# YangXiaocui1215/MGNNS

Measured on AMD Instinct MI355X. Metric: forward samples/sec at batch 256 (3-channel GCN + fusion), higher is better.
Workload: dtype bf16; 1 GPU; mvsa_multiple_b256: B=256/GPU, T=100, V=20154, 8 heads x 2 layers, C=(80,365), fp32 feature maps [B,2048,14,14] resident in HBM; global_batch=256, parallelism=batch-shard x1, launch=hipGraph replay [segments] x 2 in flight (own buffers, round robin, no join), attention=faithful, forwards_in_flight=2, schedule=place_bank_first

## Files before the change

include/mgnns_hip.h:

```cpp
#ifndef MGNNS_HIP_H
#define MGNNS_HIP_H

#include <stddef.h>
#include <stdint.h>

#ifdef __cplusplus
extern "C" {
#endif

typedef void* mgnns_stream_t;
typedef struct mgnns_comm_s* mgnns_comm_t;

#define MGNNS_ACT_NONE   0
#define MGNNS_ACT_RELU   1
#define MGNNS_ACT_LRELU2 2

#define MGNNS_ERR_ARG     (-1)
#define MGNNS_ERR_LAUNCH  (-2)
#define MGNNS_ERR_UNSUPP  (-3)

#define MGNNS_STATUS_LABEL_GCN_TIMEOUT 1
#define MGNNS_STATUS_CLUSTER_TIMEOUT   2
#define MGNNS_STATUS_BAD_PLAN          3
int mgnns_set_status_word(int32_t* host_pinned);
int mgnns_take_status(void);

const char* mgnns_last_error(void);
#define MGNNS_ABI_VERSION 26
int mgnns_abi_version(void);
const char* mgnns_source_fingerprint(void);
int mgnns_xcd_probe(int32_t* out9);

int mgnns_textgcn_fwd(const int64_t* tok, int B, int T,
                      const float* node_hidden, int V, int D,
                      const float* edge_w, int n_edge_w,
                      const int32_t* pmi_row_ptr, const int32_t* pmi_col, const int32_t* pmi_eid,
                      int ngram, int max_length, float* out, mgnns_stream_t stream);
int mgnns_textgcn_set_form(int form);

int mgnns_embedding_fwd(const int64_t* idx, int64_t n, const float* table, int V, int D,
                        float* out, mgnns_stream_t stream);

size_t mgnns_bilstm_workspace_bytes(int B, int T, int hidden, int num_layers);
int mgnns_bilstm_fwd(const int64_t* tok, const int64_t* lens, int B, int T,
                     const float* emb_table, int V, int emb_dim, int hidden, int num_layers,
                     const float* const* w_ih_cat, const float* const* b_ih_cat,
                     const float* const* w_hh, const float* const* b_hh,
                     void* workspace, size_t workspace_bytes, float* out, void* out_bf16, int ld_bf16,
                     mgnns_stream_t stream);
int mgnns_bilstm_bf16_fwd(const int64_t* tok, const int64_t* lens, int B, int T,
                     const float* emb_table, int V, int emb_dim, int hidden, int num_layers,
                     const float* const* w_ih_cat, const float* const* b_ih_cat,
                     const float* const* w_hh, const float* const* b_hh,
                     void* workspace, size_t workspace_bytes, float* out, void* out_bf16, int ld_bf16, const void* prepacked,
                     mgnns_stream_t stream);
size_t mgnns_bilstm_bf16_prepack_bytes(int hidden, int num_layers);
int mgnns_bilstm_bf16_prepack(const float* const* w_ih_cat, const float* const* w_hh, int emb_dim, int hidden, int num_layers,
                              void* packed, mgnns_stream_t stream);
size_t mgnns_bilstm_bf16_table_bytes(int V, int hidden);
size_t mgnns_bilstm_bf16_fold_workspace_bytes(int V);
int mgnns_bilstm_bf16_fold_embedding(const float* emb_table, int V, int emb_dim, int hidden, const float* w_ih_cat0,
                                     const float* b_ih_cat0, void* workspace, size_t workspace_bytes, float* table,
                                     mgnns_stream_t stream);
int mgnns_bilstm_bf16_table_fwd(const int64_t* tok, const int64_t* lens, int B, int T,
                     const float* emb_table, int V, int emb_dim, int hidden, int num_layers,
                     const float* const* w_ih_cat, const float* const* b_ih_cat,
                     const float* const* w_hh, const float* const* b_hh,
                     void* workspace, size_t workspace_bytes, float* out, void* out_bf16, int ld_bf16, const void* prepacked,
                     const float* gx_table, mgnns_stream_t stream);

int mgnns_gen_adj(const float* A, int C, float* adj, float* work ,
                  int32_t* csr_row_ptr, int32_t* csr_col, float* csr_val, mgnns_stream_t stream);

int mgnns_dense_to_csr(const float* M, int C, int32_t* csr_row_ptr, int32_t* csr_col, float* csr_val,
                       mgnns_stream_t stream);

int mgnns_matmul_fwd(const float* X, int M, int K, const float* W, int N, float* Y, int act,
                     void* workspace, size_t workspace_bytes, mgnns_stream_t stream);
int mgnns_spmm_csr_fwd(const int32_t* row_ptr, const int32_t* col, const float* val, int n_rows,
                       const float* X, int F, float* Y, int act, mgnns_stream_t stream);
int mgnns_spmm_csr_bias_fwd(const int32_t* row_ptr, const int32_t* col, const float* val, int n_rows,
                            const float* X, int F, const float* bias, float* Y, int act, mgnns_stream_t stream);

int mgnns_cast_bf16(const float* src, long long n, void* dst_bf16, mgnns_stream_t stream);
int mgnns_spmm_csr_bf16_fwd(const int32_t* row_ptr, const int32_t* col, const void* val_bf16, int n_rows, int nnz,
                            const void* X_bf16, int F, void* Y, int y_bf16, int act, int variant,
                            const int32_t* row_map, mgnns_stream_t stream);
int mgnns_spmm_tiled_bf16_fwd(const uint32_t* wave_off, const uint32_t* ent, int lane_bytes, int rows_per_wave,
                              int tile_cols, int n_rows, int n_cols, const void* X_bf16, int F, void* Y, int y_bf16,
                              int act, mgnns_stream_t stream);

int mgnns_linear_fwd(const float* X, int M, int K, const float* W, const float* bias, int N,
                     const float* residual, float* Y, int act,
                     void* workspace, size_t workspace_bytes, mgnns_stream_t stream);
size_t mgnns_gemm_workspace_bytes(void);

int mgnns_imgbank_pool_fwd(const float* feat, int B, int K, int P,
                           const float* Wt, int ldw, const float* bias, int N,
                           float* bank, float* pooled, mgnns_stream_t stream);
int mgnns_imgbank_set_form(int form);
size_t mgnns_imgbank_packed_weight_bytes(int K);
int mgnns_imgbank_pack_weights_bf16(const float* W, int N, int K, void* Wp, mgnns_stream_t stream);
int mgnns_imgbank_pool_bf16_fwd(const float* feat, int B, int K, int P, const void* Wp, const float* bias, int N,
                                void* bank_bf16, int ld, float* pooled, float* pooled_work, mgnns_stream_t stream);

int mgnns_imgbank_pool_split_fwd(const float* feat, int B, int K, int P, const void* Wp_hi, const void* Wp_lo,
                                 const float* bias, int N, float* bank, float* pooled_halves, void* bank_hi, void* bank_lo,
                                 mgnns_stream_t stream);

int mgnns_transpose_pad(const float* in, int rows, int cols, float* out, int ld, mgnns_stream_t stream);

int mgnns_label_attn_core_fwd(const float* Q, const float* K, const float* V, int B, int NLQ,
                              int n_heads, int dh, float* x, mgnns_stream_t stream);
int mgnns_label_attn_core_masked_fwd(const float* Q, const float* K, const float* V, const unsigned char* mask,
                                     int B, int NLQ, int n_heads, int dh, float* x, mgnns_stream_t stream);

int mgnns_label_tail_fwd(const float* x, int B, int C, const float* pooled, int n_parts, int K_pool,
                         const float* g_wp, const float* Q, int NLQ, int n_heads, int dh,
                         const float* wk_wp, const float* bk, const float* wv_wp, const float* bv,
                         const float* wc_wp, const float* bc, int N5, const float* xl_wp, const float* bxl,
                         int n_out, float* out, const float* wq_next_wp, const float* bq_next, int HK_next,
                         float* qh_next, mgnns_stream_t stream);

int mgnns_label_tail_bf16_fwd(const float* pooled, int B, int n_parts, int K_pool, int C, int terms,
                              const void* const* packed, const float* Q, int NLQ, int n_heads, int dh, const float* bk,
                              const float* bv, const float* bc, int N5, const float* bxl, int n_out, float* out,
                              const float* bq_next, int HK_next, float* qh_next, float* cluster_scratch,
                              int* cluster_counters, mgnns_stream_t stream);

int mgnns_sq_mha_core_fwd(const float* qh, const float* bank, const float* mask,
                          int B, int L, int D, int H, int dk,
                          const float* Wk, const float* bk, const float* Wv, const float* bv,
                          float* o, float* attn, mgnns_stream_t stream);

int mgnns_head_diff_fwd(const float* o, int B, int H, int dv, float* out, mgnns_stream_t stream);

size_t mgnns_sq_mha_packed_weight_bytes(int H);
int mgnns_sq_mha_pack_weights_bf16(const float* Wk, const float* Wv, int H, int dk, int D, void* Wp,
                                   mgnns_stream_t stream);
int mgnns_cast_pad_bf16(const float* x, int64_t rows, int D, int ld, void* y, mgnns_stream_t stream);
int mgnns_sq_mha_core_bf16_fwd(const float* qh, const void* bank_bf16, const float* mask,
                               int B, int L, int ld, int H, int dk,
                               const void* Wp, const float* bk, const float* bv,
                               float* o, float* attn, mgnns_stream_t stream);

size_t mgnns_sq_mha32_packed_weight_bytes(int H);
int mgnns_sq_mha32_pack_weights_bf16(const float* Wk, const float* Wv, int H, int dk, int D, void* Wp,
                                     mgnns_stream_t stream);
size_t mgnns_sq_mha32_plan_ints(int B);
int mgnns_sq_mha32_plan(const float* mask, int B, int L, int32_t* plan, mgnns_stream_t stream);
int mgnns_sq_mha32_core_bf16_fwd(const float* qh, const void* bank_bf16, const float* mask,
                                 int B, int L, int ld, int H, int dk,
                                 const void* Wp, const float* bk, const float* bv,
                                 float* o, float* attn, const int32_t* plan, mgnns_stream_t stream);

size_t mgnns_sq_mha_split_packed_weight_bytes(int H);
int mgnns_sq_mha_pack_weights_split(const float* Wk, const float* Wv, int H, int dk, int D, void* Wp,
                                    mgnns_stream_t stream);
int mgnns_split_pad_bf16(const float* x, int64_t rows, int D, int ld, void* hi, void* lo, mgnns_stream_t stream);
int mgnns_sq_mha_core_split_fwd(const float* qh, const void* bank_hi, const void* bank_lo, const float* mask,
                                int B, int L, int ld, int H, int dk,
                                const void* Wp, const float* bk, const float* bv,
                                float* o, float* attn, const int32_t* plan, mgnns_stream_t stream);
int mgnns_sq_mha_split_plan(const float* mask, int B, int L, int32_t* plan, mgnns_stream_t stream);

size_t mgnns_sq_mha_folded_workspace_bytes(int B, int D, int H);
int mgnns_sq_mha_folded_fwd(const float* qh, const void* bank, int bank_is_bf16, int ld_bank, const float* mask,
                            int B, int L, int D, int H, int dk, const float* Wk, const float* Wv, const float* bv,
                            void* workspace, size_t workspace_bytes, float* o, float* attn, mgnns_stream_t stream);

int mgnns_sq_mha_folded_bf16_fwd(const float* U, const void* bank_bf16, const float* mask, int B, int L, int D, int H,
                                 float inv_temp, void* C_bf16, int ldc, float* attn, mgnns_stream_t stream);

size_t mgnns_packed_f32_weight_bytes(int N, int K);
int mgnns_pack_weight_f32(const float* W, int N, int K, float* Wp, mgnns_stream_t stream);
int mgnns_mha_tail_fwd(const float* o, int HK, const float* q, int B, int d_model,
                       const float* fc_wp, const float* fc_b, const float* ln1_gamma, const float* ln1_beta,
                       const float* w1_wp, const float* b1, const float* w2_wp, const float* b2,
                       const float* ln2_gamma, const float* ln2_beta, float eps, float* out,
                       const float* wq_next_wp, const float* bq_next, int HK_next, float* qh_next,
                       mgnns_stream_t stream);

size_t mgnns_packed_bf16_weight_bytes(int N, int K);
int mgnns_pack_weight_bf16_split(const float* W, int N, int K, void* Whi, void* Wlo, mgnns_stream_t stream);
int mgnns_mha_tail_bf16_fwd(const float* o, int HK, const float* q, int B, int d_model, int terms,
                            const void* const* packed,
                            const float* fc_b, const float* ln1_gamma, const float* ln1_beta, const float* b1,
                            const float* b2, const float* ln2_gamma, const float* ln2_beta, float eps, float* out,
                            const float* bq_next, int HK_next, float* qh_next, int cluster, float* cluster_scratch,
                            int* cluster_counters, mgnns_stream_t stream);

size_t mgnns_mha_tail_c16_scratch_floats(int B, int cluster);
int mgnns_mha_tail_c16_fwd(const void* c_bf16, int HC, const float* q, int B, int d_model, const void* const* packed,
                           const float* fc_b, const float* ln1_gamma, const float* ln1_beta, const float* b1,
                           const float* b2, const float* ln2_gamma, const float* ln2_beta, float eps, float* out,
                           const float* bq_next, int HC_next, float* u_next, int cluster, float* cluster_scratch,
                           int* cluster_counters, mgnns_stream_t stream);

int mgnns_label_gcn_supported(int C, int K0, int N1, int N2, int split);
int mgnns_label_tail_supported(int C, int NLQ, int n_heads, int dh, int N5, int n_out, int K_pool, int with_next_q);
int mgnns_label_tail_bf16_supported(int C, int NLQ, int n_heads, int dh, int N5, int n_out, int K_pool, int terms, int with_next_q);
size_t mgnns_label_gcn_scratch_bytes(int C, int N1, int N2);
int mgnns_label_gcn_fwd(const float* A, int C, const float* inp, int K0, int split, const void* w1a, const void* w1b, int N1,
                        const void* w2a, const void* w2b, int N2, float* G, void* Gp_hi, void* Gp_lo,
                        const float* label_query, int NLQ, const float* wq, const float* bq, int HQ, float* Q,
                        void* scratch, size_t scratch_bytes, int grid, mgnns_stream_t stream);
size_t mgnns_label_gcn_memo_bytes(int C, int K0);
int mgnns_label_gcn_memo_fwd(const float* A, int C, const float* inp, int K0, int split, const void* w1a, const void* w1b, int N1,
                             const void* w2a, const void* w2b, int N2, float* G, void* Gp_hi, void* Gp_lo,
                             const float* label_query, int NLQ, const float* wq, const float* bq, int HQ, float* Q,
                             void* scratch, size_t scratch_bytes, void* memo, size_t memo_bytes, int grid, mgnns_stream_t stream);

int mgnns_classifier_head_fwd(const float* f0, const float* f1, const float* f2, const float* f3, int B, int D,
                              const float* W, const float* bias, int NL, float* logits, mgnns_stream_t stream);
int mgnns_classifier_part_fwd(const float* f, int part, int nparts, int B, int D, const float* W, const float* bias,
                              int NL, float* parts, int* counter, float* logits, mgnns_stream_t stream);

int mgnns_layernorm_fwd(const float* x, int rows, int D, const float* gamma, const float* beta,
                        float eps, float* y, mgnns_stream_t stream);

int mgnns_mha_train_fwd(const float* qh, const float* bank, const float* mask, int B, int L, int D, int H, int dk,
                        const float* Wk, const float* Wv, const float* bv, uint64_t seed, float rate, float* U, float* P,
                        float* attn, uint8_t* keep, float* Z, float* SP, float* o, mgnns_stream_t stream);
size_t mgnns_mha_train_bwd_workspace_bytes(int B, int D, int H, int dk);
int mgnns_mha_train_bwd(const float* dO, const float* qh, const float* bank, const float* mask, int B, int L, int D, int H,
                        int dk, const float* Wk, const float* Wv, const float* bv, float rate, const float* U, const float* P,
                        const float* attn, const uint8_t* keep, const float* Z, const float* SP, float* dqh, float* dWk,
                        float* dWv, float* dbv, float* dbank, void* workspace, size_t workspace_bytes, mgnns_stream_t stream);
size_t mgnns_wgrad_workspace_bytes(int M, int N, int K);
int mgnns_wgrad_fwd(const float* dY, int M, int N, const float* X, int K, float* dW, float* db, void* workspace,
                    size_t workspace_bytes, mgnns_stream_t stream);
int mgnns_drop_res_ln_fwd(const float* x, const float* res, int rows, int D, const float* gamma, const float* beta, float eps,
                          uint64_t seed, int site, float rate, float* y, float* xhat, float* sig, uint8_t* keep,
                          mgnns_stream_t stream);
int mgnns_drop_res_ln_bwd(const float* dy, const float* dy2, const float* xhat, const float* sig, const uint8_t* keep, int rows,
                          int D, const float* gamma, float eps, float rate, float* dres, float* dx, float* dgamma, float* dbeta,
                          mgnns_stream_t stream);
#define MGNNS_ELT_ADD        0
#define MGNNS_ELT_RELU_BWD   1
#define MGNNS_ELT_LRELU2_BWD 2
int mgnns_train_eltwise(int op, const float* a, const float* b, int64_t n, float* y, mgnns_stream_t stream);

#define MGNNS_DROP_LABEL_ATTN 3
#define MGNNS_DROP_HEAD       4
size_t mgnns_imgbank_wgrad_workspace_bytes(int B, int K, int P, int N);
int mgnns_imgbank_wgrad(const float* X, const float* dbank, int B, int K, int P, int N, float* dW, float* db, void* workspace,
                        size_t workspace_bytes, mgnns_stream_t stream);
int mgnns_map_argmax(const float* X, int B, int K, int P, int32_t* arg, mgnns_stream_t stream);
int mgnns_imgbank_dgrad(const float* dbank, const float* W, const float* dpooled, const int32_t* arg, int B, int K, int P, int N,
                        float* dX, mgnns_stream_t stream);
size_t mgnns_imgbank_wgrad_split_workspace_bytes(int B, int K, int P, int N);
int mgnns_imgbank_wgrad_split(const float* X, const float* dbank, int B, int K, int P, int N, float* dW, float* db,
                              void* workspace, size_t workspace_bytes, mgnns_stream_t stream);
size_t mgnns_imgbank_dgrad_split_workspace_bytes(int B, int K, int P, int N);
int mgnns_imgbank_dgrad_split(const float* dbank, const float* W, const float* dpooled, const int32_t* arg, int B, int K, int P,
                              int N, float* dX, void* workspace, size_t workspace_bytes, mgnns_stream_t stream);
int mgnns_label_attn_train_fwd(const float* Q, const float* K, const float* V, int B, int NLQ, int H, int dh, uint64_t seed,
                               float rate, float* x, float* P, uint8_t* keep, mgnns_stream_t stream);
size_t mgnns_label_attn_train_bwd_workspace_bytes(int B, int NLQ, int H, int dh);
int mgnns_label_attn_train_bwd(const float* dx, const float* Q, const float* K, const float* V, const float* P,
                               const uint8_t* keep, int B, int NLQ, int H, int dh, float rate, float* dQ, float* dK, float* dV,
                               void* workspace, size_t workspace_bytes, mgnns_stream_t stream);

#define MGNNS_DROP_LSTM       5
#define MGNNS_DROP_TEXT_GCN   6
size_t mgnns_bilstm_train_workspace_bytes(int B, int T, int hidden);
int mgnns_bilstm_train_fwd(const int64_t* tok, const int64_t* lens, int B, int T, const float* emb_table, int V, int emb_dim,
                           int hidden, int num_layers, const float* const* w_ih_cat, const float* const* b_ih_cat,
                           const float* const* w_hh, const float* const* b_hh, uint64_t seed, float rate, int32_t* meta,
                           int rows_cap, float* gates, float* cells, float* mid, float* mid_drop, float* out, void* workspace,
                           size_t workspace_bytes, mgnns_stream_t stream);
int mgnns_bilstm_train_bwd_rec(const float* dout, const int64_t* lens, int B, int T, const int32_t* meta, int rows_cap,
                               const float* gates, const float* cells, const float* w_hh_f, const float* w_hh_r, float* dz,
                               mgnns_stream_t stream);
int mgnns_bilstm_train_hprev(const float* hout, const int64_t* lens, int B, int T, const int32_t* meta, int rows_cap, float* hprev,
                             mgnns_stream_t stream);
int mgnns_bilstm_train_unpack_drop(const float* dx, const int32_t* pack_pos, int64_t M, int B, int T, uint64_t seed, float rate,
                                   float* dout, mgnns_stream_t stream);
int mgnns_gather_rows(const float* src, int n_src, int K, const int32_t* idx, int64_t M, float* dst, mgnns_stream_t stream);
int mgnns_keyed_row_sum(const int64_t* sorted_keys, const int64_t* perm, int64_t M, const float* values, int D, int64_t n_values,
                        int64_t skip_below, float* out, int64_t K, mgnns_stream_t stream);
int mgnns_textgcn_train_fwd(const int64_t* tok, int B, int T, const float* node_hidden, int V, int D, const float* edge_w,
                            int n_edge_w, const int32_t* pmi_row_ptr, const int32_t* pmi_col, const int32_t* pmi_eid, int ngram,
                            int max_length, uint64_t seed, float rate, float* out, float* presum, int16_t* win,
                            mgnns_stream_t stream);
int mgnns_textgcn_train_bwd(const int64_t* tok, int B, int T, const float* node_hidden, int V, int D, const float* edge_w,
                            int n_edge_w, const int32_t* pmi_row_ptr, const int32_t* pmi_col, const int32_t* pmi_eid, int ngram,
                            int max_length, uint64_t seed, float rate, const float* dy, const float* presum, const int16_t* win,
                            float* R, int32_t* keyR, float* Eg, int32_t* keyE, mgnns_stream_t stream);
int mgnns_dropout_fwd(const float* x, int64_t n, uint64_t seed, int site, float rate, float* y, uint8_t* keep,
                      mgnns_stream_t stream);
int mgnns_dropout_bwd(const float* dy, const uint8_t* keep, int64_t n, float rate, float* dx, mgnns_stream_t stream);
int mgnns_dropout_mask(uint64_t seed, int site, float rate, int64_t n, uint8_t* keep, mgnns_stream_t stream);

int mgnns_transpose_cast_bf16(const float* x, int rows, int cols, int ld, void* y, mgnns_stream_t stream);
size_t mgnns_gemm_bf16_workspace_bytes(void);
int mgnns_gemm_bf16_nt_fwd(const void* A, const void* Bt, int M, int N, int Kp, const float* bias, void* C, int ldc,
                           int c_bf16, int act, void* workspace, size_t workspace_bytes, mgnns_stream_t stream);
int mgnns_gemm_bf16_set_form(int form);
int mgnns_gemm_bf16_pick_form(int M, int N, int Kp, int with_workspace, int n_cu);

int mgnns_softmax_argmax_fwd(const float* logits, int B, int NL, float* probs, int32_t* pred, const int64_t* target,
                             int32_t* confusion, mgnns_stream_t stream);

int mgnns_conv_fold_bn_bf16(const float* w, const float* conv_bias, int Cout, int Cin, int KH, int KW,
                            const float* gamma, const float* beta, const float* mean, const float* var, float eps,
                            int k_order, int ld, void* wt, float* bias, mgnns_stream_t stream);
int mgnns_stem_conv7_fwd(const float* img, int B, int H, int W, const void* wt, const float* bias, void* y,
                         mgnns_stream_t stream);
int mgnns_maxpool3x3s2_nhwc_fwd(const void* x, int B, int H, int W, int C, void* y, mgnns_stream_t stream);
int mgnns_conv_bf16_nhwc_fwd(const void* x, int B, int H, int W, int Cin, const void* wt, const float* bias, int Cout,
                             int KH, int KW, int stride, int pad, const void* residual, int relu, int out_nchw_f32,
                             void* y, mgnns_stream_t stream);

int mgnns_conv_transpose_pack_bf16(const void* wt, int Cout, int Cin, int KH, int KW, void* wT, mgnns_stream_t stream);
int mgnns_conv_dgrad_bf16_nhwc(const void* dy, int B, int H, int W, int Cin, const void* wT, int Cout, int KH, int KW,
                               int stride, int pad, const void* mask, const void* add, void* dx, mgnns_stream_t stream);
size_t mgnns_conv_wgrad_workspace_bytes(int B, int H, int W, int Cin, int Cout, int KH, int KW, int stride, int pad);
int mgnns_conv_wgrad_bf16_nhwc(const void* x, const void* dy, int B, int H, int W, int Cin, int Cout, int KH, int KW,
                               int stride, int pad, float* dW, float* db, void* workspace, size_t workspace_bytes,
                               mgnns_stream_t stream);
int mgnns_conv_bn_unfold(const float* dWp, const float* dbp, const float* w, const float* gamma, const float* mean,
                         const float* var, float eps, int Cout, int Cin, int KH, int KW, float* dW, float* dgamma,
                         float* dbeta, mgnns_stream_t stream);
int mgnns_map_grad_relu_nhwc_bf16(const float* map, const float* dmap, int B, int C, int P, void* g, mgnns_stream_t stream);

size_t mgnns_bn_stats_workspace_bytes(int M, int C);
int mgnns_bn_stats_bf16(const void* z, int M, int C, float eps, double momentum, float* mean, float* rstd, float* var,
                        float* running_mean, float* running_var, void* workspace, size_t workspace_bytes,
                        mgnns_stream_t stream);
int mgnns_bn_apply_bf16(const void* z, int M, int C, const float* mean, const float* rstd, const float* gamma,
                        const float* beta, const void* residual, int relu, int out_nchw_f32, int P, void* y,
                        mgnns_stream_t stream);
size_t mgnns_bn_backward_workspace_bytes(int M, int C);
int mgnns_bn_backward_bf16(const void* g, const void* z, int M, int C, const float* mean, const float* rstd,
                           const float* gamma, void* gz, float* dgamma, float* dbeta, void* workspace,
                           size_t workspace_bytes, mgnns_stream_t stream);

int mgnns_debug_stamp(uint64_t* slots, int idx, mgnns_stream_t stream);

int mgnns_debug_slabcopy(const void* src, void* dst, int n_rows, int pitch, int piece, int mode, int wgx,
                         mgnns_stream_t stream);

int mgnns_debug_spin(int microseconds, uint64_t* slots, int idx, mgnns_stream_t stream);

int mgnns_comm_unique_id(void* id, size_t bytes );
int mgnns_comm_init_rank(int world, int rank, const void* id, size_t bytes, mgnns_comm_t* comm);
int mgnns_comm_init_all(int ndev, const int* devices, mgnns_comm_t* comms);
int mgnns_comm_info(mgnns_comm_t comm, int* world, int* rank);
int mgnns_allgather_logits(mgnns_comm_t comm, const float* local, int rows_local, int num_labels, float* all,
                           mgnns_stream_t stream);
int mgnns_comm_group_start(void);
int mgnns_comm_group_end(void);
int mgnns_comm_destroy(mgnns_comm_t comm);

#ifdef __cplusplus
}
#endif
#endif
```

mgnns_amd/_lib.py:

```python
import ctypes
import os

_HERE = os.path.dirname(os.path.abspath(__file__))
LIB_PATH = os.environ.get("MGNNS_LIB") or os.path.join(_HERE, "libmgnns_hip.so")
ABI_VERSION = 26

_c = ctypes
_P = _c.c_void_p
_I = _c.c_int
_L = _c.c_int64
_F = _c.c_float
_SZ = _c.c_size_t
_U64 = _c.c_uint64
_PP = _c.POINTER(_c.c_void_p)

SIGNATURES = {
    "mgnns_textgcn_fwd": [_P, _I, _I, _P, _I, _I, _P, _I, _P, _P, _P, _I, _I, _P, _P],
    "mgnns_bilstm_fwd": [_P, _P, _I, _I, _P, _I, _I, _I, _I, _PP, _PP, _PP, _PP, _P, _SZ, _P, _P, _I, _P],
    "mgnns_bilstm_bf16_fwd": [_P, _P, _I, _I, _P, _I, _I, _I, _I, _PP, _PP, _PP, _PP, _P, _SZ, _P, _P, _I, _P, _P],
    "mgnns_bilstm_bf16_prepack": [_PP, _PP, _I, _I, _I, _P, _P],
    "mgnns_bilstm_bf16_fold_embedding": [_P, _I, _I, _I, _P, _P, _P, _SZ, _P, _P],
    "mgnns_bilstm_bf16_table_fwd": [_P, _P, _I, _I, _P, _I, _I, _I, _I, _PP, _PP, _PP, _PP, _P, _SZ, _P, _P, _I, _P, _P, _P],
    "mgnns_embedding_fwd": [_P, _L, _P, _I, _I, _P, _P],
    "mgnns_gen_adj": [_P, _I, _P, _P, _P, _P, _P, _P],
    "mgnns_dense_to_csr": [_P, _I, _P, _P, _P, _P],
    "mgnns_matmul_fwd": [_P, _I, _I, _P, _I, _P, _I, _P, _SZ, _P],
    "mgnns_spmm_csr_fwd": [_P, _P, _P, _I, _P, _I, _P, _I, _P],
    "mgnns_spmm_csr_bias_fwd": [_P, _P, _P, _I, _P, _I, _P, _P, _I, _P],
    "mgnns_cast_bf16": [_P, _c.c_longlong, _P, _P],
    "mgnns_spmm_csr_bf16_fwd": [_P, _P, _P, _I, _I, _P, _I, _P, _I, _I, _I, _P, _P],
    "mgnns_spmm_tiled_bf16_fwd": [_P, _P, _I, _I, _I, _I, _I, _P, _I, _P, _I, _I, _P],
    "mgnns_linear_fwd": [_P, _I, _I, _P, _P, _I, _P, _P, _I, _P, _SZ, _P],
    "mgnns_imgbank_pool_fwd": [_P, _I, _I, _I, _P, _I, _P, _I, _P, _P, _P],
    "mgnns_imgbank_pack_weights_bf16": [_P, _I, _I, _P, _P],
    "mgnns_imgbank_pool_bf16_fwd": [_P, _I, _I, _I, _P, _P, _I, _P, _I, _P, _P, _P],
    "mgnns_imgbank_set_form": [_I],
    "mgnns_textgcn_set_form": [_I],
    "mgnns_head_diff_fwd": [_P, _I, _I, _I, _P, _P],
    "mgnns_classifier_part_fwd": [_P, _I, _I, _I, _I, _P, _P, _I, _P, _P, _P, _P],
    "mgnns_imgbank_pool_split_fwd": [_P, _I, _I, _I, _P, _P, _P, _I, _P, _P, _P, _P, _P],
    "mgnns_transpose_pad": [_P, _I, _I, _P, _I, _P],
    "mgnns_label_attn_core_fwd": [_P, _P, _P, _I, _I, _I, _I, _P, _P],
    "mgnns_label_attn_core_masked_fwd": [_P, _P, _P, _P, _I, _I, _I, _I, _P, _P],
    "mgnns_label_gcn_fwd": [_P, _I, _P, _I, _I, _P, _P, _I, _P, _P, _I, _P, _P, _P, _P, _I, _P, _P, _I, _P, _P, _SZ, _I, _P],
    "mgnns_label_gcn_memo_fwd": [_P, _I, _P, _I, _I, _P, _P, _I, _P, _P, _I, _P, _P, _P, _P, _I, _P, _P, _I, _P, _P, _SZ, _P, _SZ, _I, _P],
    "mgnns_classifier_head_fwd": [_P, _P, _P, _P, _I, _I, _P, _P, _I, _P, _P],
    "mgnns_label_tail_bf16_fwd": [_P, _I, _I, _I, _I, _I, _PP, _P, _I, _I, _I, _P, _P, _P, _I, _P, _I, _P, _P, _I, _P, _P, _P, _P],
    "mgnns_label_tail_fwd": [_P, _I, _I, _P, _I, _I, _P, _P, _I, _I, _I, _P, _P, _P, _P, _P, _P, _I, _P, _P, _I, _P, _P, _P,
                             _I, _P, _P],
    "mgnns_sq_mha_core_fwd": [_P, _P, _P, _I, _I, _I, _I, _I, _P, _P, _P, _P, _P, _P, _P],
    "mgnns_sq_mha_pack_weights_bf16": [_P, _P, _I, _I, _I, _P, _P],
    "mgnns_cast_pad_bf16": [_P, _L, _I, _I, _P, _P],
    "mgnns_sq_mha_core_bf16_fwd": [_P, _P, _P, _I, _I, _I, _I, _I, _P, _P, _P, _P, _P, _P],
    "mgnns_sq_mha32_pack_weights_bf16": [_P, _P, _I, _I, _I, _P, _P],
    "mgnns_sq_mha32_plan": [_P, _I, _I, _P, _P],
    "mgnns_sq_mha32_core_bf16_fwd": [_P, _P, _P, _I, _I, _I, _I, _I, _P, _P, _P, _P, _P, _P, _P],
    "mgnns_sq_mha_pack_weights_split": [_P, _P, _I, _I, _I, _P, _P],
    "mgnns_split_pad_bf16": [_P, _L, _I, _I, _P, _P, _P],
    "mgnns_sq_mha_core_split_fwd": [_P, _P, _P, _P, _I, _I, _I, _I, _I, _P, _P, _P, _P, _P, _P, _P],
    "mgnns_sq_mha_split_plan": [_P, _I, _I, _P, _P],
    "mgnns_sq_mha_folded_fwd": [_P, _P, _I, _I, _P, _I, _I, _I, _I, _I, _P, _P, _P, _P, _SZ, _P, _P, _P],
    "mgnns_pack_weight_f32": [_P, _I, _I, _P, _P],
    "mgnns_mha_tail_fwd": [_P, _I, _P, _I, _I, _P, _P, _P, _P, _P, _P, _P, _P, _P, _P, _F, _P, _P, _P, _I, _P, _P],
    "mgnns_pack_weight_bf16_split": [_P, _I, _I, _P, _P, _P],
    "mgnns_mha_tail_bf16_fwd": [_P, _I, _P, _I, _I, _I, _PP, _P, _P, _P, _P, _P, _P, _P, _F, _P, _P, _I, _P, _I, _P, _P, _P],
    "mgnns_mha_tail_c16_fwd": [_P, _I, _P, _I, _I, _PP, _P, _P, _P, _P, _P, _P, _P, _F, _P, _P, _I, _P, _I, _P, _P, _P],
    "mgnns_sq_mha_folded_bf16_fwd": [_P, _P, _P, _I, _I, _I, _I, _F, _P, _I, _P, _P],
    "mgnns_transpose_cast_bf16": [_P, _I, _I, _I, _P, _P],
    "mgnns_gemm_bf16_nt_fwd": [_P, _P, _I, _I, _I, _P, _P, _I, _I, _I, _P, _SZ, _P],
    "mgnns_gemm_bf16_set_form": [_I],
    "mgnns_gemm_bf16_pick_form": [_I, _I, _I, _I, _I],
    "mgnns_softmax_argmax_fwd": [_P, _I, _I, _P, _P, _P, _P, _P],
    "mgnns_conv_fold_bn_bf16": [_P, _P, _I, _I, _I, _I, _P, _P, _P, _P, _F, _I, _I, _P, _P, _P],
    "mgnns_stem_conv7_fwd": [_P, _I, _I, _I, _P, _P, _P, _P],
    "mgnns_maxpool3x3s2_nhwc_fwd": [_P, _I, _I, _I, _I, _P, _P],
    "mgnns_conv_bf16_nhwc_fwd": [_P, _I, _I, _I, _I, _P, _P, _I, _I, _I, _I, _I, _P, _I, _I, _P, _P],
    "mgnns_conv_transpose_pack_bf16": [_P, _I, _I, _I, _I, _P, _P],
    "mgnns_conv_dgrad_bf16_nhwc": [_P, _I, _I, _I, _I, _P, _I, _I, _I, _I, _I, _P, _P, _P, _P],
    "mgnns_conv_wgrad_bf16_nhwc": [_P, _P, _I, _I, _I, _I, _I, _I, _I, _I, _I, _P, _P, _P, _SZ, _P],
    "mgnns_conv_bn_unfold": [_P, _P, _P, _P, _P, _P, _F, _I, _I, _I, _I, _P, _P, _P, _P],
    "mgnns_map_grad_relu_nhwc_bf16": [_P, _P, _I, _I, _I, _P, _P],
    "mgnns_bn_stats_bf16": [_P, _I, _I, _F, _c.c_double, _P, _P, _P, _P, _P, _P, _SZ, _P],
    "mgnns_bn_apply_bf16": [_P, _I, _I, _P, _P, _P, _P, _P, _I, _I, _I, _P, _P],
    "mgnns_bn_backward_bf16": [_P, _P, _I, _I, _P, _P, _P, _P, _P, _P, _P, _SZ, _P],
    "mgnns_label_gcn_supported": [_I, _I, _I, _I, _I],
    "mgnns_label_tail_supported": [_I, _I, _I, _I, _I, _I, _I, _I],
    "mgnns_label_tail_bf16_supported": [_I, _I, _I, _I, _I, _I, _I, _I, _I],
    "mgnns_xcd_probe": [_P],
    "mgnns_set_status_word": [_P],
    "mgnns_take_status": [],
    "mgnns_debug_slabcopy": [_P, _P, _I, _I, _I, _I, _I, _P],
    "mgnns_debug_stamp": [_P, _I, _P],
    "mgnns_debug_spin": [_I, _P, _I, _P],
    "mgnns_layernorm_fwd": [_P, _I, _I, _P, _P, _F, _P, _P],
    "mgnns_mha_train_fwd": [_P, _P, _P, _I, _I, _I, _I, _I, _P, _P, _P, _U64, _F, _P, _P, _P, _P, _P, _P, _P, _P],
    "mgnns_mha_train_bwd": [_P, _P, _P, _P, _I, _I, _I, _I, _I, _P, _P, _P, _F, _P, _P, _P, _P, _P, _P, _P, _P, _P, _P, _P,
                            _P, _SZ, _P],
    "mgnns_wgrad_fwd": [_P, _I, _I, _P, _I, _P, _P, _P, _SZ, _P],
    "mgnns_drop_res_ln_fwd": [_P, _P, _I, _I, _P, _P, _F, _U64, _I, _F, _P, _P, _P, _P, _P],
    "mgnns_drop_res_ln_bwd": [_P, _P, _P, _P, _P, _I, _I, _P, _F, _F, _P, _P, _P, _P, _P],
    "mgnns_train_eltwise": [_I, _P, _P, _L, _P, _P],
    "mgnns_imgbank_wgrad": [_P, _P, _I, _I, _I, _I, _P, _P, _P, _SZ, _P],
    "mgnns_map_argmax": [_P, _I, _I, _I, _P, _P],
    "mgnns_imgbank_dgrad": [_P, _P, _P, _P, _I, _I, _I, _I, _P, _P],
    "mgnns_imgbank_wgrad_split": [_P, _P, _I, _I, _I, _I, _P, _P, _P, _SZ, _P],
    "mgnns_imgbank_dgrad_split": [_P, _P, _P, _P, _I, _I, _I, _I, _P, _P, _SZ, _P],
    "mgnns_label_attn_train_fwd": [_P, _P, _P, _I, _I, _I, _I, _U64, _F, _P, _P, _P, _P],
    "mgnns_label_attn_train_bwd": [_P, _P, _P, _P, _P, _P, _I, _I, _I, _I, _F, _P, _P, _P, _P, _SZ, _P],
    "mgnns_dropout_fwd": [_P, _L, _U64, _I, _F, _P, _P, _P],
    "mgnns_dropout_bwd": [_P, _P, _L, _F, _P, _P],
    "mgnns_dropout_mask": [_U64, _I, _F, _L, _P, _P],
    "mgnns_bilstm_train_fwd": [_P, _P, _I, _I, _P, _I, _I, _I, _I, _PP, _PP, _PP, _PP, _U64, _F, _P, _I, _P, _P, _P, _P, _P, _P,
                               _SZ, _P],
    "mgnns_bilstm_train_bwd_rec": [_P, _P, _I, _I, _P, _I, _P, _P, _P, _P, _P, _P],
    "mgnns_bilstm_train_hprev": [_P, _P, _I, _I, _P, _I, _P, _P],
    "mgnns_bilstm_train_unpack_drop": [_P, _P, _L, _I, _I, _U64, _F, _P, _P],
    "mgnns_gather_rows": [_P, _I, _I, _P, _L, _P, _P],
    "mgnns_keyed_row_sum": [_P, _P, _L, _P, _I, _L, _L, _P, _L, _P],
    "mgnns_textgcn_train_fwd": [_P, _I, _I, _P, _I, _I, _P, _I, _P, _P, _P, _I, _I, _U64, _F, _P, _P, _P, _P],
    "mgnns_textgcn_train_bwd": [_P, _I, _I, _P, _I, _I, _P, _I, _P, _P, _P, _I, _I, _U64, _F, _P, _P, _P, _P, _P, _P, _P, _P],
    "mgnns_comm_unique_id": [_P, _SZ],
    "mgnns_comm_init_rank": [_I, _I, _P, _SZ, _PP],
    "mgnns_comm_init_all": [_I, _P, _PP],
    "mgnns_comm_info": [_P, _c.POINTER(_I), _c.POINTER(_I)],
    "mgnns_allgather_logits": [_P, _P, _I, _I, _P, _P],
    "mgnns_comm_group_start": [],
    "mgnns_comm_group_end": [],
    "mgnns_comm_destroy": [_P],
}

SIZE_GETTERS = {
    "mgnns_packed_bf16_weight_bytes": [_I, _I],
    "mgnns_packed_f32_weight_bytes": [_I, _I],
    "mgnns_gemm_workspace_bytes": [],
    "mgnns_gemm_bf16_workspace_bytes": [],
    "mgnns_imgbank_packed_weight_bytes": [_I],
    "mgnns_sq_mha_packed_weight_bytes": [_I],
    "mgnns_sq_mha32_packed_weight_bytes": [_I],
    "mgnns_sq_mha32_plan_ints": [_I],
    "mgnns_sq_mha_split_packed_weight_bytes": [_I],
    "mgnns_sq_mha_folded_workspace_bytes": [_I, _I, _I],
    "mgnns_bilstm_workspace_bytes": [_I, _I, _I, _I],
    "mgnns_bilstm_bf16_prepack_bytes": [_I, _I],
    "mgnns_bilstm_bf16_table_bytes": [_I, _I],
    "mgnns_bilstm_bf16_fold_workspace_bytes": [_I],
    "mgnns_label_gcn_scratch_bytes": [_I, _I, _I],
    "mgnns_label_gcn_memo_bytes": [_I, _I],
    "mgnns_mha_tail_c16_scratch_floats": [_I, _I],
    "mgnns_mha_train_bwd_workspace_bytes": [_I, _I, _I, _I],
    "mgnns_wgrad_workspace_bytes": [_I, _I, _I],
    "mgnns_imgbank_wgrad_workspace_bytes": [_I, _I, _I, _I],
    "mgnns_imgbank_wgrad_split_workspace_bytes": [_I, _I, _I, _I],
    "mgnns_imgbank_dgrad_split_workspace_bytes": [_I, _I, _I, _I],
    "mgnns_label_attn_train_bwd_workspace_bytes": [_I, _I, _I, _I],
    "mgnns_bilstm_train_workspace_bytes": [_I, _I, _I],
    "mgnns_conv_wgrad_workspace_bytes": [_I, _I, _I, _I, _I, _I, _I, _I, _I],
    "mgnns_bn_stats_workspace_bytes": [_I, _I],
    "mgnns_bn_backward_workspace_bytes": [_I, _I],
}

_lib = None


class MgnnsLibraryError(RuntimeError):
    pass


def lib():
    global _lib
    if _lib is not None:
        return _lib
    if not os.path.exists(LIB_PATH):
        raise MgnnsLibraryError(
            "%s is missing: the HIP extension is mandatory (no CPU/PyTorch fallback exists). "
            "Build it with `python -m mgnns_amd.build`." % LIB_PATH)
    import torch
    L = ctypes.CDLL(LIB_PATH)
    L.mgnns_last_error.restype = ctypes.c_char_p
    L.mgnns_last_error.argtypes = []
    L.mgnns_abi_version.restype = _I
    L.mgnns_abi_version.argtypes = []
    L.mgnns_source_fingerprint.restype = ctypes.c_char_p
    L.mgnns_source_fingerprint.argtypes = []
    if L.mgnns_abi_version() != ABI_VERSION:
        raise MgnnsLibraryError("libmgnns_hip.so ABI %d != binding ABI %d; rebuild" % (L.mgnns_abi_version(), ABI_VERSION))
    for name, args in SIZE_GETTERS.items():
        fn = getattr(L, name)
        fn.restype = _SZ
        fn.argtypes = args
    for name, args in SIGNATURES.items():
        fn = getattr(L, name)
        fn.restype = _I
        fn.argtypes = args
    _lib = L
    _register_status_word(L)
    return L


def source_state():
    from . import build
    built, tree = lib().mgnns_source_fingerprint().decode(), build.source_fingerprint()
    return built, tree, built == tree


def check_sources(who="this measurement"):
    built, tree, same = source_state()
    if not same:
        raise MgnnsLibraryError("%s: %s was built from sources %s, the tree holds %s -- rebuild (python -m mgnns_amd.build) first"
                                % (who, LIB_PATH, built, tree))
    return built


_status_word = None


def _register_status_word(L):
    global _status_word
    import torch
    if _status_word is not None or not torch.cuda.is_available():
        return
    try:
        w = torch.zeros(16, dtype=torch.int32).pin_memory()
    except RuntimeError:
        return
    L.mgnns_set_status_word(w.data_ptr())
    _status_word = w


def xcd_probe():
    import ctypes
    out = (ctypes.c_int32 * 9)()
    check(lib().mgnns_xcd_probe(ctypes.addressof(out)), "mgnns_xcd_probe")
    return bool(out[0]), [int(out[1 + k]) for k in range(8)]


def take_status():
    code = lib().mgnns_take_status()
    if code:
        raise RuntimeError("a launch raised the library status word (status %d: 1 / 2 = a persistent launch gave up a bounded wait, "
                           "3 = a masked attention launch refused its plan): results since then are invalid" % code)


def check(rc, name):
    if rc != 0:
        raise RuntimeError("%s failed (%d): %s" % (name, rc, lib().mgnns_last_error().decode()))
```

mgnns_amd/csrc/label_tail.hip:

```cpp
#include "common.hpp"
#include "tile_f32.hpp"

namespace {

constexpr int LT_THR = 512;
constexpr int LT_ROWS = 16;
constexpr int LT_MAXKQ = 20;
constexpr int LT_MAXH = 8;

__host__ __device__ inline int lt_stride(int k) {
    const int kp = (k + 15) / 16 * 16;
    return kp + ((34 - (kp % 32)) % 32);
}

constexpr int LT_KCH = 512;

__global__ __launch_bounds__(LT_THR) void label_tail_kernel(const float* __restrict__ x, int B, int C,
                                                            const float* __restrict__ pooled, int n_parts, int KP,
                                                            const float* __restrict__ g_wp,
                                                            const float* __restrict__ Q, int NLQ, int n_heads, int dh,
                                                            const float* __restrict__ wk_wp, const float* __restrict__ bk,
                                                            const float* __restrict__ wv_wp, const float* __restrict__ bv,
                                                            const float* __restrict__ wc_wp, const float* __restrict__ bc, int N5,
                                                            const float* __restrict__ xl_wp, const float* __restrict__ bxl, int NO,
                                                            float* __restrict__ out, const float* __restrict__ wq_wp,
                                                            const float* __restrict__ bq, int HKn, float* __restrict__ qh_next) {
    extern __shared__ __attribute__((aligned(16))) float smem[];
    const int hid = n_heads * dh;
    const int sx = lt_stride(C), sh = lt_stride(hid), sf = lt_stride(NLQ * N5);
    float* s_x = smem;
    float* s_k = s_x + LT_ROWS * sx;
    float* s_v = s_k + LT_ROWS * sh;
    float* s_o = s_v + LT_ROWS * sh;
    float* s_f = s_o + LT_ROWS * sh;
    float* s_q = s_f + LT_ROWS * sf;
    const int tid = threadIdx.x, lane = tid & 63, wave = tid >> 6;
    const int r0 = blockIdx.x * LT_ROWS;
    const int crow = (lane >> 4) * 4, ccol = lane & 15;
    const int NTh = (hid + 15) / 16, NT5 = (N5 + 15) / 16, NTo = (NO + 15) / 16;
    const int KQh = (hid + 15) / 16;

    f32x4 wc[LT_MAXKQ];
    if (wave < NT5) {
#pragma unroll
        for (int kq = 0; kq < LT_MAXKQ; ++kq)
            wc[kq] = kq < KQh ? reinterpret_cast<const f32x4*>(wc_wp)[((size_t)wave * KQh + kq) * 64 + lane] : f32x4{0.f, 0.f, 0.f, 0.f};
    }
    for (int i = tid; i < LT_ROWS * sx + 3 * LT_ROWS * sh + LT_ROWS * sf; i += LT_THR) s_x[i] = 0.f;
    for (int i = tid; i < NLQ * hid; i += LT_THR) s_q[i] = Q[i];
    __syncthreads();
    if (g_wp) {
        const int NTc = (C + 15) / 16, KQ = (KP + 15) / 16;
        const int sp = lt_stride(LT_KCH);
        float* s_p = s_f;
        for (int t0 = 0; t0 * 8 < NTc; t0 += 3) {
            f32x4 acc[3] = {f32x4{0.f, 0.f, 0.f, 0.f}, f32x4{0.f, 0.f, 0.f, 0.f}, f32x4{0.f, 0.f, 0.f, 0.f}};
            for (int k0 = 0; k0 < KP; k0 += LT_KCH) {
                const int kn = min(LT_KCH, KP - k0);
                for (int i = tid; i < LT_ROWS * (LT_KCH / 4); i += LT_THR) {
                    const int r = i / (LT_KCH / 4), c4 = (i - r * (LT_KCH / 4)) * 4;
                    f32x4 v = {0.f, 0.f, 0.f, 0.f};
                    if (r0 + r < B && c4 < kn) {
                        const float* src = pooled + ((size_t)(r0 + r) * n_parts) * KP + k0 + c4;
                        v = *reinterpret_cast<const f32x4*>(src);
                        for (int pt = 1; pt < n_parts; ++pt) {
                            const f32x4 u = *reinterpret_cast<const f32x4*>(src + (size_t)pt * KP);
                            v = f32x4{fmaxf(v.x, u.x), fmaxf(v.y, u.y), fmaxf(v.z, u.z), fmaxf(v.w, u.w)};
                        }
                    }
                    float* d = s_p + r * sp + c4;
                    *reinterpret_cast<float2*>(d) = float2{v.x, v.y};
                    *reinterpret_cast<float2*>(d + 2) = float2{v.z, v.w};
                }
                __syncthreads();
                mg_tile_gemm_f32_chunk<3>(acc, s_p, sp, k0 / 16, (k0 + kn + 15) / 16, KQ, g_wp, NTc, wave, lane, t0);
                __syncthreads();
            }
#pragma unroll
            for (int t = 0; t < 3; ++t) {
                const int nt = wave + 8 * (t0 + t), n = nt * 16 + ccol;
                if (nt < NTc && n < C) {
#pragma unroll
                    for (int r = 0; r < 4; ++r) s_x[(crow + r) * sx + n] = acc[t][r];
                }
            }
        }
        for (int i = tid; i < LT_ROWS * sf; i += LT_THR) s_f[i] = 0.f;
    } else {
        for (int i = tid; i < LT_ROWS * C; i += LT_THR) {
            const int r = i / C, c = i - r * C;
            if (r0 + r < B) s_x[r * sx + c] = x[(size_t)(r0 + r) * C + c];
        }
    }
    __syncthreads();

    for (int t0 = 0; t0 * 8 < NTh; t0 += 3) {
        f32x4 ak[3], av[3];
        mg_tile_gemm_f32<3>(ak, s_x, sx, C, wk_wp, NTh, wave, lane, t0);
        mg_tile_gemm_f32<3>(av, s_x, sx, C, wv_wp, NTh, wave, lane, t0);
#pragma unroll
        for (int t = 0; t < 3; ++t) {
            const int nt = wave + 8 * (t0 + t), n = nt * 16 + ccol;
            if (nt < NTh && n < hid) {
                const float b0 = bk[n], b1 = bv[n];
#pragma unroll
                for (int r = 0; r < 4; ++r) {
                    s_k[(crow + r) * sh + n] = ak[t][r] + b0;
                    s_v[(crow + r) * sh + n] = av[t][r] + b1;
                }
            }
        }
    }
    __syncthreads();

    const float inv_scale = 1.0f / sqrtf((float)dh);
    for (int l = 0; l < NLQ; ++l) {
#pragma unroll 1
        for (int rr = 0; rr < 2; ++rr) {
            const int r = 2 * wave + rr;
            const bool on = lane < dh;
            float e[LT_MAXH], vv[LT_MAXH];
#pragma unroll
            for (int h = 0; h < LT_MAXH; ++h) {
                const int c = (h < n_heads ? h : 0) * dh + (on ? lane : 0);
                e[h] = (on && h < n_heads) ? s_q[l * hid + c] * s_k[r * sh + c] * inv_scale : -INFINITY;
                vv[h] = s_v[r * sh + c];
            }
#pragma unroll
            for (int h = 0; h < LT_MAXH; ++h) {
                if (h < n_heads) {
                    const float m = wave_max_dpp(e[h]);
                    const float p = on ? expf(e[h] - m) : 0.f;
                    const float z = wave_sum_dpp(p);
                    if (on) s_o[r * sh + h * dh + lane] = (p / z) * vv[h];
                }
            }
        }
        __syncthreads();
        if (wave < NT5) {
            f32x4 acc = {0.f, 0.f, 0.f, 0.f};
            const float* ap = s_o + (lane & 15) * sh + (lane >> 4);
#pragma unroll
            for (int kq = 0; kq < LT_MAXKQ; ++kq) {
                if (kq < KQh) {
#pragma unroll
                    for (int j = 0; j < 4; ++j) acc = __builtin_amdgcn_mfma_f32_16x16x4f32(ap[(4 * kq + j) * 4], wc[kq][j], acc, 0, 0, 0);
                }
            }
            const int n = wave * 16 + ccol;
            if (n < N5) {
                const float b0 = bc[n];
#pragma unroll
                for (int r = 0; r < 4; ++r) s_f[(crow + r) * sf + l * N5 + n] = acc[r] + b0;
            }
        }
        __syncthreads();
    }

    for (int t0 = 0; t0 * 8 < NTo; t0 += 3) {
        f32x4 acc[3];
        mg_tile_gemm_f32<3>(acc, s_f, sf, NLQ * N5, xl_wp, NTo, wave, lane, t0);
#pragma unroll
        for (int t = 0; t < 3; ++t) {
            const int nt = wave + 8 * (t0 + t), n = nt * 16 + ccol;
            if (nt < NTo && n < NO) {
                const float b0 = bxl[n];
#pragma unroll
                for (int r = 0; r < 4; ++r) {
                    const int gr = r0 + crow + r;
                    const float v = acc[t][r] + b0;
                    if (gr < B) out[(size_t)gr * NO + n] = v;
                    if (wq_wp) s_o[(crow + r) * sh + n] = v;
                }
            }
        }
    }
    if (wq_wp) {
        __syncthreads();
        const int NTq = (HKn + 15) / 16;
        for (int t0 = 0; t0 * 8 < NTq; t0 += 3) {
            f32x4 acc[3];
            mg_tile_gemm_f32<3>(acc, s_o, sh, NO, wq_wp, NTq, wave, lane, t0);
#pragma unroll
            for (int t = 0; t < 3; ++t) {
                const int nt = wave + 8 * (t0 + t), n = nt * 16 + ccol;
                if (nt < NTq && n < HKn) {
                    const float b0 = bq ? bq[n] : 0.f;
#pragma unroll
                    for (int r = 0; r < 4; ++r) {
                        const int gr = r0 + crow + r;
                        if (gr < B) qh_next[(size_t)gr * HKn + n] = acc[t][r] + b0;
                    }
                }
            }
        }
    }
}

}

extern "C" int mgnns_label_tail_supported(int C, int NLQ, int n_heads, int dh, int N5, int n_out, int K_pool, int with_next_q) {
    if (!(C > 0 && NLQ > 0 && n_heads > 0 && dh > 0 && dh <= 64 && N5 > 0 && n_out > 0)) return 0;
    if (K_pool && K_pool % 4) return 0;
    const int hid = n_heads * dh;
    if (!(hid <= 16 * LT_MAXKQ && n_heads <= LT_MAXH && N5 <= 128)) return 0;
    if (with_next_q && n_out != hid) return 0;
    if (K_pool && lt_stride(NLQ * N5) < lt_stride(LT_KCH)) return 0;
    const size_t lds = ((size_t)LT_ROWS * (lt_stride(C) + 3 * lt_stride(hid) + lt_stride(NLQ * N5)) + (size_t)NLQ * hid) * sizeof(float);
    return lds <= 160 * 1024 ? 1 : 0;
}

extern "C" int mgnns_label_tail_fwd(const float* x, int B, int C, const float* pooled, int n_parts, int K_pool,
                                    const float* g_wp, const float* Q, int NLQ, int n_heads, int dh,
                                    const float* wk_wp, const float* bk, const float* wv_wp, const float* bv,
                                    const float* wc_wp, const float* bc, int N5, const float* xl_wp, const float* bxl,
                                    int n_out, float* out, const float* wq_next_wp, const float* bq_next, int HK_next,
                                    float* qh_next, mgnns_stream_t stream) {
    MG_REQUIRE(B >= 0 && C > 0 && NLQ > 0 && n_heads > 0 && dh > 0 && dh <= 64 && N5 > 0 && n_out > 0,
               "mgnns_label_tail_fwd: bad dims B=%d C=%d NLQ=%d heads=%d dh=%d N5=%d out=%d", B, C, NLQ, n_heads, dh, N5, n_out);
    if (B == 0) return 0;
    MG_REQUIRE(Q && wk_wp && bk && wv_wp && bv && wc_wp && bc && xl_wp && bxl && out, "mgnns_label_tail_fwd: null pointer");
    MG_REQUIRE((x != nullptr) != (g_wp != nullptr), "mgnns_label_tail_fwd: pass EITHER the read-out x OR pooled + packed G");
    if (g_wp) {
        MG_REQUIRE(pooled && n_parts >= 1 && K_pool > 0 && K_pool % 4 == 0 && mg_aligned16(pooled),
                   "mgnns_label_tail_fwd: pooled [B,%d,%d] must be 16-byte aligned with K %% 4 == 0", n_parts, K_pool);
    }
    const int hid = n_heads * dh;
    MG_REQUIRE(hid <= 16 * LT_MAXKQ && n_heads <= LT_MAXH, "mgnns_label_tail_fwd: hidden width %d / %d heads unsupported (<= %d, <= %d)",
               hid, n_heads, 16 * LT_MAXKQ, LT_MAXH);
    MG_REQUIRE(N5 <= 128, "mgnns_label_tail_fwd: linear_5 width %d unsupported (<= 128)", N5);
    MG_REQUIRE(!wq_next_wp || (qh_next && HK_next > 0 && n_out == hid),
               "mgnns_label_tail_fwd: the query projection needs qh_next, HK_next and n_out == hidden width");
    const int sfl = lt_stride(NLQ * N5) > lt_stride(LT_KCH) || !g_wp ? lt_stride(NLQ * N5) : lt_stride(LT_KCH);
    MG_REQUIRE(!g_wp || lt_stride(NLQ * N5) >= lt_stride(LT_KCH), "mgnns_label_tail_fwd: NLQ*N5=%d too small to stage the read-out (>= %d)",
               NLQ * N5, LT_KCH);
    (void)sfl;
    const size_t lds = ((size_t)LT_ROWS * (lt_stride(C) + 3 * lt_stride(hid) + lt_stride(NLQ * N5)) + (size_t)NLQ * hid) * sizeof(float);
    MG_REQUIRE(lds <= 160 * 1024, "mgnns_label_tail_fwd: C=%d, NLQ*N5=%d need %zu B of LDS (> 160 KiB)", C, NLQ * N5, lds);
    MG_DYN_LDS(label_tail_kernel, 160 * 1024);
    hipLaunchKernelGGL(label_tail_kernel, dim3((B + LT_ROWS - 1) / LT_ROWS), dim3(LT_THR), lds, (hipStream_t)stream, x, B, C,
                       pooled, n_parts, K_pool, g_wp, Q, NLQ, n_heads, dh, wk_wp, bk, wv_wp, bv, wc_wp, bc, N5, xl_wp, bxl, n_out,
                       out, wq_next_wp, bq_next, HK_next, qh_next);
    MG_CHECK_LAUNCH("mgnns_label_tail_fwd");
    return 0;
}

#include "tile_bf16.hpp"

#ifdef MG_LT_TRACE
__device__ unsigned long long g_lt_trace[16];
#define LT_STAMP(i) do { if (threadIdx.x == 0 && blockIdx.x == 0) g_lt_trace[i] = __builtin_amdgcn_s_memtime(); } while (0)
extern "C" int mgnns_debug_lt_trace(unsigned long long* out) {
    return hipMemcpyFromSymbol(out, HIP_SYMBOL(g_lt_trace), sizeof(unsigned long long) * 16) == hipSuccess ? 0 : 1;
}
#else
#define LT_STAMP(i) do { } while (0)
#endif

namespace {

constexpr int LB_MAXKS = 10;

struct LabelW {
    const unsigned short *g_h, *g_l, *wk_h, *wk_l, *wv_h, *wv_l, *wc_h, *wc_l, *xl_h, *xl_l, *wq_h, *wq_l;
    const float *bk, *bv, *bc, *bxl, *bq;
};

__device__ __forceinline__ unsigned pk2(float a, float b) { return mg_bf16(a) | (unsigned)mg_bf16(b) << 16; }

template <int TERMS, int CL>
__global__ __launch_bounds__(LT_THR) void label_tail_bf16_kernel(const float* __restrict__ pooled, int B, int n_parts, int KP, int C,
                                                                 const float* __restrict__ Q, int NLQ, int n_heads, int dh,
                                                                 LabelW w, int N5, int NO, float* __restrict__ out, int HKn,
                                                                 float* __restrict__ qh_next, float* __restrict__ xpart,
                                                                 int* __restrict__ counters, int* __restrict__ status) {
    extern __shared__ __attribute__((aligned(16))) unsigned char smem_b[];
    constexpr int NH = TERMS == 3 ? 4 : 1;
    constexpr int LO = TERMS == 3 ? 1 : 0;
    const int hid = n_heads * dh;
    const int KSp = KP / 32, KSpp = KSp / NH, KSx = (C + 31) / 32, KSh = (hid + 31) / 32, KSf = (NLQ * N5 + 31) / 32;
    const int sp = 4 * KSpp + 2, sxc = 4 * KSx + 2, shc = 4 * KSh + 2, sfc = 4 * KSf + 2;
    const int shf = lt_stride(hid);
    const int spf = sp > sfc ? sp : sfc;
    uint4* s_ph = reinterpret_cast<uint4*>(smem_b);
    uint4* s_pl = s_ph + LT_ROWS * spf;
    uint4* s_xh = s_pl + LO * LT_ROWS * spf;
    uint4* s_xl = s_xh + LT_ROWS * sxc;
    uint4* s_oh = s_xl + LO * LT_ROWS * sxc;
    uint4* s_ol = s_oh + LT_ROWS * shc;
    float* s_k = reinterpret_cast<float*>(s_ol + LO * LT_ROWS * shc);
    float* s_v = s_k + LT_ROWS * shf;
    float* s_q = s_v + LT_ROWS * shf;
    uint4* s_fh = s_ph;
    uint4* s_fl = s_pl;
    if (!LO) { s_pl = s_ph; s_xl = s_xh; s_ol = s_oh; s_fl = s_fh; }
    const int tid = threadIdx.x, lane = tid & 63, wave = tid >> 6;
    const int tile = (int)blockIdx.x / CL, crank = (int)blockIdx.x % CL;
    const int r0 = tile * LT_ROWS;
    const int crow = (lane >> 4) * 4, ccol = lane & 15;
    const int NTc = (C + 15) / 16, NTh = (hid + 15) / 16, NT5 = (N5 + 15) / 16, NTo = (NO + 15) / 16;
    unsigned short* xh16 = reinterpret_cast<unsigned short*>(s_xh);
    unsigned short* xl16 = reinterpret_cast<unsigned short*>(s_xl);
    unsigned short* oh16 = reinterpret_cast<unsigned short*>(s_oh);
    unsigned short* ol16 = reinterpret_cast<unsigned short*>(s_ol);
    unsigned short* fh16 = reinterpret_cast<unsigned short*>(s_fh);
    unsigned short* fl16 = reinterpret_cast<unsigned short*>(s_fl);
    auto put = [&](unsigned short* h, unsigned short* l, int idx, float v) {
        if (LO) mg_split_store(h, l, idx, v); else h[idx] = mg_bf16(v);
    };

    LT_STAMP(0);
#ifndef MG_LT_TOUCH
#define MG_LT_TOUCH 0
#endif
#ifndef MG_LT_PF3
#define MG_LT_PF3 4
#endif
    WRing<3, TERMS, (TERMS == 3 ? MG_LT_PF3 : 10)> ring;
    ring_prime(ring, KSpp, w.g_h, w.g_l, NTc, wave, lane, 0, KSp, CL > 1 ? crank * KSpp : 0);
#if MG_LT_TOUCH
    int touch_sink = 0;
    {
        auto touch = [&](const unsigned short* base, int nt_n, int ks_total, int ks_lo, int ks_n, int nt_lo = 0) {
            if (!base || nt_n <= 0) return;
            base += ((size_t)nt_lo * ks_total) << 9;
            const int lines = nt_n * ks_n * 8;
            for (int i = tid; i < lines; i += LT_THR) {
                const int nt = i / (ks_n * 8), rem = i - nt * (ks_n * 8);
                const char* p = reinterpret_cast<const char*>(base) + ((size_t)(nt * ks_total + ks_lo + (rem >> 3)) << 10) + ((rem & 7) << 7);
                asm volatile("global_load_dword %0, %1, off" : "+v"(touch_sink) : "v"(p) : "memory");
            }
        };
        const int NTq_ = (HKn + 15) / 16;
        touch(w.g_h, NTc, KSp, CL > 1 ? crank * KSpp : 0, CL > 1 ? KSpp : KSp);
        if (LO) touch(w.g_l, NTc, KSp, CL > 1 ? crank * KSpp : 0, CL > 1 ? KSpp : KSp);
        touch(w.wk_h, NTh, KSx, 0, KSx);
        if (LO) touch(w.wk_l, NTh, KSx, 0, KSx);
        touch(w.wv_h, NTh, KSx, 0, KSx);
        if (LO) touch(w.wv_l, NTh, KSx, 0, KSx);
        touch(w.wc_h, NT5, KSh, 0, KSh);
        if (LO) touch(w.wc_l, NT5, KSh, 0, KSh);
        touch(w.xl_h, NTo, KSf, 0, KSf);
        if (LO) touch(w.xl_l, NTo, KSf, 0, KSf);
        const int qs_ = (NTq_ + 7) / 8, qp_ = (qs_ + CL - 1) / CL;
        const int qt_lo = crank * qp_ * 8, qt_hi = (crank * qp_ + qp_) * 8 < NTq_ ? (crank * qp_ + qp_) * 8 : NTq_;
        touch(w.wq_h, qt_hi - qt_lo, KSh, 0, KSh, qt_lo);
        if (LO) touch(w.wq_l, qt_hi - qt_lo, KSh, 0, KSh, qt_lo);
    }
#endif
    for (int i = tid; i < (1 + LO) * LT_ROWS * (sxc + shc); i += LT_THR) s_xh[i] = make_uint4(0u, 0u, 0u, 0u);
    for (int i = tid; i < 2 * LT_ROWS * shf; i += LT_THR) s_k[i] = 0.f;
    for (int i = tid; i < NLQ * hid; i += LT_THR) s_q[i] = Q[i];

    f32x4 acc[3];
    LT_STAMP(1);
    static_assert(CL == 1 || CL == NH, "a cluster rank owns one K part of the read-out");
    for (int hpart = CL > 1 ? crank : 0; hpart < (CL > 1 ? crank + 1 : NH); ++hpart) {
        const int kq8 = KP / NH / 8;
        for (int i = tid; i < LT_ROWS * kq8; i += LT_THR) {
            const int r = i / kq8, c8 = i - r * kq8;
            f32x4 a = {0.f, 0.f, 0.f, 0.f}, b = a;
            if (r0 + r < B) {
                const float* src = pooled + ((size_t)(r0 + r) * n_parts) * KP + hpart * (KP / NH) + 8 * c8;
                a = *reinterpret_cast<const f32x4*>(src);
                b = *reinterpret_cast<const f32x4*>(src + 4);
                for (int pt = 1; pt < n_parts; ++pt) {
                    const f32x4 u = *reinterpret_cast<const f32x4*>(src + (size_t)pt * KP);
                    const f32x4 v = *reinterpret_cast<const f32x4*>(src + (size_t)pt * KP + 4);
                    a = f32x4{fmaxf(a.x, u.x), fmaxf(a.y, u.y), fmaxf(a.z, u.z), fmaxf(a.w, u.w)};
                    b = f32x4{fmaxf(b.x, v.x), fmaxf(b.y, v.y), fmaxf(b.z, v.z), fmaxf(b.w, v.w)};
                }
            }
            s_ph[r * sp + c8] = make_uint4(pk2(a.x, a.y), pk2(a.z, a.w), pk2(b.x, b.y), pk2(b.z, b.w));
            if (LO) {
                auto lo = [](float x) { return x - mg_bf16_f32(mg_bf16(x)); };
                s_pl[r * sp + c8] = make_uint4(pk2(lo(a.x), lo(a.y)), pk2(lo(a.z), lo(a.w)), pk2(lo(b.x), lo(b.y)), pk2(lo(b.z), lo(b.w)));
            }
        }
        __syncthreads();
        if (CL == 1 && hpart) ring_prime(ring, KSpp, w.g_h, w.g_l, NTc, wave, lane, 0, KSp, hpart * KSpp);
        ring_gemm(acc, ring, s_ph, s_pl, sp, KSpp, w.g_h, w.g_l, lane, CL == 1 && hpart != 0);
        __syncthreads();
    }
    LT_STAMP(2);
    ring_prime(ring, KSx, w.wk_h, w.wk_l, NTh, wave, lane, 0);
    if (CL > 1) {
        const __amdgpu_buffer_rsrc_t xp = mg_buffer(xpart + (size_t)tile * CL * (8 * 3 * 64 * 4), CL * 8 * 3 * 64 * 16);
        const int slot = (wave * 3 * 64 + lane) * 16;
#pragma unroll
        for (int t = 0; t < 3; ++t)
            if (wave + 8 * t < NTc)
                __builtin_amdgcn_raw_buffer_store_b128(__builtin_bit_cast(i32x4, acc[t]), xp, slot + t * 64 * 16, crank * (8 * 3 * 64 * 16), 17);
        asm volatile("s_waitcnt vmcnt(0)" ::: "memory");
        __syncthreads();
        if (tid == 0) {
            __hip_atomic_fetch_add(&counters[2 * tile], 1, __ATOMIC_RELAXED, __HIP_MEMORY_SCOPE_AGENT);
            int spins = 0;
            while (__hip_atomic_load(&counters[2 * tile], __ATOMIC_RELAXED, __HIP_MEMORY_SCOPE_AGENT) < CL) {
                if (++spins > (1 << 24)) {
                    if (status) __hip_atomic_store(status, MGNNS_STATUS_CLUSTER_TIMEOUT, __ATOMIC_RELAXED, __HIP_MEMORY_SCOPE_SYSTEM);
                    break;
                }
                __builtin_amdgcn_s_sleep(4);
            }
        }
        __syncthreads();
#pragma unroll
        for (int t = 0; t < 3; ++t) {
            f32x4 pr[CL];
#pragma unroll
            for (int rk = 0; rk < CL; ++rk)
                pr[rk] = wave + 8 * t < NTc ? __builtin_bit_cast(f32x4, __builtin_amdgcn_raw_buffer_load_b128(xp, slot + t * 64 * 16, rk * (8 * 3 * 64 * 16), 17))
                                            : f32x4{0.f, 0.f, 0.f, 0.f};
            acc[t] = pr[0];
#pragma unroll
            for (int rk = 1; rk < CL; ++rk) acc[t] += pr[rk];
        }
    }
#pragma unroll
    for (int t = 0; t < 3; ++t) {
        const int nt = wave + 8 * t, n = nt * 16 + ccol;
        if (nt < NTc && n < C) {
#pragma unroll
            for (int r = 0; r < 4; ++r) put(xh16, xl16, (crow + r) * sxc * 8 + n, acc[t][r]);
        }
    }
    for (int i = tid; i < (1 + LO) * LT_ROWS * spf; i += LT_THR) s_ph[i] = make_uint4(0u, 0u, 0u, 0u);
    __syncthreads();
    if (CL > 1 && tid == 0) {
        const int old = __hip_atomic_fetch_add(&counters[2 * tile + 1], 1, __ATOMIC_RELAXED, __HIP_MEMORY_SCOPE_AGENT);
        if (old == CL - 1) {
            __hip_atomic_store(&counters[2 * tile], 0, __ATOMIC_RELAXED, __HIP_MEMORY_SCOPE_AGENT);
            __hip_atomic_store(&counters[2 * tile + 1], 0, __ATOMIC_RELAXED, __HIP_MEMORY_SCOPE_AGENT);
        }
    }
    LT_STAMP(3);
    ring_gemm(acc, ring, s_xh, s_xl, sxc, KSx, w.wk_h, w.wk_l, lane);
    ring_prime(ring, KSx, w.wv_h, w.wv_l, NTh, wave, lane, 0);
#pragma unroll
    for (int t = 0; t < 3; ++t) {
        const int nt = wave + 8 * t, n = nt * 16 + ccol;
        if (nt < NTh && n < hid) {
            const float b0 = w.bk[n];
#pragma unroll
            for (int r = 0; r < 4; ++r) s_k[(crow + r) * shf + n] = acc[t][r] + b0;
        }
    }
    ring_gemm(acc, ring, s_xh, s_xl, sxc, KSx, w.wv_h, w.wv_l, lane);
    ring_prime(ring, KSf, w.xl_h, w.xl_l, NTo, wave, lane, 0);
#pragma unroll
    for (int t = 0; t < 3; ++t) {
        const int nt = wave + 8 * t, n = nt * 16 + ccol;
        if (nt < NTh && n < hid) {
            const float b0 = w.bv[n];
#pragma unroll
            for (int r = 0; r < 4; ++r) s_v[(crow + r) * shf + n] = acc[t][r] + b0;
        }
    }
    uint4 wch[LB_MAXKS], wcl[LO ? LB_MAXKS : 1];
    if (wave < NT5) {
#pragma unroll
        for (int ks = 0; ks < LB_MAXKS; ++ks) {
            const size_t off = ((size_t)wave * KSh + (ks < KSh ? ks : 0)) * 64 + lane;
            wch[ks] = reinterpret_cast<const uint4*>(w.wc_h)[off];
            if (LO) wcl[ks] = reinterpret_cast<const uint4*>(w.wc_l)[off];
        }
    }
    __syncthreads();

    const float inv_scale = 1.0f / sqrtf((float)dh);
    LT_STAMP(4);
    for (int l = 0; l < NLQ; ++l) {
#pragma unroll 1
        for (int rr = 0; rr < 2; ++rr) {
            const int r = 2 * wave + rr;
            const bool on = lane < dh;
            float e[LT_MAXH], vv[LT_MAXH];
#pragma unroll
            for (int h = 0; h < LT_MAXH; ++h) {
                const int c = (h < n_heads ? h : 0) * dh + (on ? lane : 0);
                e[h] = (on && h < n_heads) ? s_q[l * hid + c] * s_k[r * shf + c] * inv_scale : -INFINITY;
                vv[h] = s_v[r * shf + c];
            }
#pragma unroll
            for (int h = 0; h < LT_MAXH; ++h) {
                if (h < n_heads) {
                    const float m = wave_max_dpp(e[h]);
                    const float p = on ? __expf(e[h] - m) : 0.f;
                    const float z = wave_sum_dpp(p);
                    if (on) put(oh16, ol16, r * shc * 8 + h * dh + lane, (p / z) * vv[h]);
                }
            }
        }
        __syncthreads();
        if (wave < NT5) {
            f32x4 a = {0.f, 0.f, 0.f, 0.f};
            const int aoff = (lane & 15) * shc + (lane >> 4);
#pragma unroll
            for (int ks = 0; ks < LB_MAXKS; ++ks)
                if (ks < KSh) {
                    const bf16x8 ah = __builtin_bit_cast(bf16x8, s_oh[aoff + ks * 4]);
                    a = __builtin_amdgcn_mfma_f32_16x16x32_bf16(ah, __builtin_bit_cast(bf16x8, wch[ks]), a, 0, 0, 0);
                    if (LO) {
                        a = __builtin_amdgcn_mfma_f32_16x16x32_bf16(ah, __builtin_bit_cast(bf16x8, wcl[ks]), a, 0, 0, 0);
                        a = __builtin_amdgcn_mfma_f32_16x16x32_bf16(__builtin_bit_cast(bf16x8, s_ol[aoff + ks * 4]),
                                                                    __builtin_bit_cast(bf16x8, wch[ks]), a, 0, 0, 0);
                    }
                }
            const int n = wave * 16 + ccol;
            if (n < N5) {
                const float b0 = w.bc[n];
#pragma unroll
                for (int r = 0; r < 4; ++r) put(fh16, fl16, (crow + r) * sfc * 8 + l * N5 + n, a[r] + b0);
            }
        }
        __syncthreads();
    }

    LT_STAMP(5);
    ring_gemm(acc, ring, s_fh, s_fl, sfc, KSf, w.xl_h, w.xl_l, lane);
    LT_STAMP(6);
    const int q_slots = ((HKn + 15) / 16 + 7) / 8, q_per = (q_slots + CL - 1) / CL;
    const int q_lo = crank * q_per, q_hi = q_lo + q_per < q_slots ? q_lo + q_per : q_slots;
    if (w.wq_h) ring_prime(ring, KSh, w.wq_h, w.wq_l, (HKn + 15) / 16, wave, lane, q_lo);
#pragma unroll
    for (int t = 0; t < 3; ++t) {
        const int nt = wave + 8 * t, n = nt * 16 + ccol;
        if (nt < NTo && n < NO) {
            const float b0 = w.bxl[n];
#pragma unroll
            for (int r = 0; r < 4; ++r) {
                const int gr = r0 + crow + r;
                const float v = acc[t][r] + b0;
                if (gr < B && crank == 0) out[(size_t)gr * NO + n] = v;
                if (w.wq_h) put(oh16, ol16, (crow + r) * shc * 8 + n, v);
            }
        }
    }
    if (w.wq_h) {
        __syncthreads();
        const int NTq = (HKn + 15) / 16;
        for (int t0 = q_lo; t0 < q_hi; t0 += 3) {
            if (t0 != q_lo) ring_prime(ring, KSh, w.wq_h, w.wq_l, NTq, wave, lane, t0);
            ring_gemm(acc, ring, s_oh, s_ol, shc, KSh, w.wq_h, w.wq_l, lane);
#pragma unroll
            for (int t = 0; t < 3; ++t) {
                const int nt = wave + 8 * (t0 + t), n = nt * 16 + ccol;
                if (t0 + t < q_hi && nt < NTq && n < HKn) {
                    const float b0 = w.bq ? w.bq[n] : 0.f;
#pragma unroll
                    for (int r = 0; r < 4; ++r) {
                        const int gr = r0 + crow + r;
                        if (gr < B) qh_next[(size_t)gr * HKn + n] = acc[t][r] + b0;
                    }
                }
            }
        }
    }
#if MG_LT_TOUCH
    asm volatile("s_waitcnt vmcnt(0)" : "+v"(touch_sink)::"memory");
#endif
    LT_STAMP(7);
}

}

extern "C" int mgnns_label_tail_bf16_supported(int C, int NLQ, int n_heads, int dh, int N5, int n_out, int K_pool, int terms,
                                               int with_next_q) {
    if (!(C > 0 && C <= 384 && NLQ > 0 && n_heads > 0 && dh > 0 && dh <= 64 && N5 > 0 && N5 <= 128 && n_out > 0)) return 0;
    if (terms != 1 && terms != 3) return 0;
    if (!(K_pool > 0 && K_pool % 128 == 0)) return 0;
    const int hid = n_heads * dh;
    if (!(hid <= 32 * LB_MAXKS && n_out <= 384 && n_heads <= LT_MAXH)) return 0;
    if (with_next_q && n_out != hid) return 0;
    const int nh = terms == 3 ? 4 : 1, lo = terms == 3 ? 1 : 0;
    const int sp = 4 * (K_pool / 32 / nh) + 2, sxc = 4 * ((C + 31) / 32) + 2, shc = 4 * ((hid + 31) / 32) + 2, sfc = 4 * ((NLQ * N5 + 31) / 32) + 2;
    const size_t lds = (size_t)(1 + lo) * LT_ROWS * ((sp > sfc ? sp : sfc) + sxc + shc) * 16 +
                       ((size_t)2 * LT_ROWS * lt_stride(hid) + (size_t)NLQ * hid) * sizeof(float);
    return lds <= 160 * 1024 ? 1 : 0;
}

extern "C" int mgnns_label_tail_bf16_fwd(const float* pooled, int B, int n_parts, int K_pool, int C, int terms,
                                         const void* const* packed ,
                                         const float* Q, int NLQ, int n_heads, int dh, const float* bk, const float* bv,
                                         const float* bc, int N5, const float* bxl, int n_out, float* out,
                                         const float* bq_next, int HK_next, float* qh_next, float* cluster_scratch,
                                         int* cluster_counters, mgnns_stream_t stream) {
    MG_REQUIRE(B >= 0 && C > 0 && C <= 384 && NLQ > 0 && n_heads > 0 && dh > 0 && dh <= 64 && N5 > 0 && N5 <= 128 && n_out > 0,
               "mgnns_label_tail_bf16_fwd: bad dims B=%d C=%d (<= 384) NLQ=%d heads=%d dh=%d N5=%d out=%d", B, C, NLQ, n_heads, dh, N5, n_out);
    MG_REQUIRE(terms == 1 || terms == 3, "mgnns_label_tail_bf16_fwd: terms must be 1 (bf16) or 3 (split-bf16)");
    if (B == 0) return 0;
    MG_REQUIRE(pooled && packed && Q && bk && bv && bc && bxl && out, "mgnns_label_tail_bf16_fwd: null pointer");
    for (int i = 0; i < 10; ++i) MG_REQUIRE(packed[i], "mgnns_label_tail_bf16_fwd: packed weight %d missing", i);
    MG_REQUIRE(n_parts >= 1 && K_pool > 0 && K_pool % 128 == 0 && mg_aligned16(pooled),
               "mgnns_label_tail_bf16_fwd: pooled [B,%d,%d] must be 16-byte aligned with K %% 128 == 0", n_parts, K_pool);
    const int hid = n_heads * dh;
    MG_REQUIRE(hid <= 32 * LB_MAXKS && n_out <= 384 && n_heads <= LT_MAXH,
               "mgnns_label_tail_bf16_fwd: hidden width %d / output width %d / %d heads unsupported", hid, n_out, n_heads);
    MG_REQUIRE(!packed[10] || (packed[11] && qh_next && HK_next > 0 && n_out == hid),
               "mgnns_label_tail_bf16_fwd: the query projection needs both packed buffers, qh_next, HK_next and n_out == hidden width");
    LabelW w;
    const unsigned short* const* pk = reinterpret_cast<const unsigned short* const*>(packed);
    w.g_h = pk[0]; w.g_l = pk[1]; w.wk_h = pk[2]; w.wk_l = pk[3]; w.wv_h = pk[4]; w.wv_l = pk[5]; w.wc_h = pk[6]; w.wc_l = pk[7];
    w.xl_h = pk[8]; w.xl_l = pk[9]; w.wq_h = pk[10]; w.wq_l = pk[11];
    w.bk = bk; w.bv = bv; w.bc = bc; w.bxl = bxl; w.bq = bq_next;
    const int nh = terms == 3 ? 4 : 1, lo = terms == 3 ? 1 : 0;
    const int sp = 4 * (K_pool / 32 / nh) + 2, sxc = 4 * ((C + 31) / 32) + 2, shc = 4 * ((hid + 31) / 32) + 2, sfc = 4 * ((NLQ * N5 + 31) / 32) + 2;
    const size_t lds = (size_t)(1 + lo) * LT_ROWS * ((sp > sfc ? sp : sfc) + sxc + shc) * 16 +
                       ((size_t)2 * LT_ROWS * lt_stride(hid) + (size_t)NLQ * hid) * sizeof(float);
    MG_REQUIRE(lds <= 160 * 1024, "mgnns_label_tail_bf16_fwd: K_pool=%d, C=%d need %zu B of LDS (> 160 KiB)", K_pool, C, lds);
    MG_REQUIRE((cluster_scratch != nullptr) == (cluster_counters != nullptr), "mgnns_label_tail_bf16_fwd: cluster scratch and counters go together");
    MG_REQUIRE(!cluster_scratch || mg_aligned16(cluster_scratch), "mgnns_label_tail_bf16_fwd: cluster scratch must be 16-byte aligned");
    if (cluster_scratch)
        if (int rc = mg_check_status("mgnns_label_tail_bf16_fwd")) return rc;
    MG_DYN_LDS((label_tail_bf16_kernel<1, 1>), 160 * 1024);
    MG_DYN_LDS((label_tail_bf16_kernel<3, 1>), 160 * 1024);
    MG_DYN_LDS((label_tail_bf16_kernel<3, 4>), 160 * 1024);
    const int tiles = (B + LT_ROWS - 1) / LT_ROWS;
    const dim3 blk(LT_THR);
    if (terms == 3 && cluster_scratch)
        hipLaunchKernelGGL((label_tail_bf16_kernel<3, 4>), dim3(tiles * 4), blk, lds, (hipStream_t)stream, pooled, B, n_parts, K_pool, C, Q, NLQ,
                           n_heads, dh, w, N5, n_out, out, HK_next, qh_next, cluster_scratch, cluster_counters, mg_status_word());
    else if (terms == 3)
        hipLaunchKernelGGL((label_tail_bf16_kernel<3, 1>), dim3(tiles), blk, lds, (hipStream_t)stream, pooled, B, n_parts, K_pool, C, Q, NLQ, n_heads, dh,
                           w, N5, n_out, out, HK_next, qh_next, (float*)nullptr, (int*)nullptr, (int*)nullptr);
    else
        hipLaunchKernelGGL((label_tail_bf16_kernel<1, 1>), dim3(tiles), blk, lds, (hipStream_t)stream, pooled, B, n_parts, K_pool, C, Q, NLQ, n_heads, dh,
                           w, N5, n_out, out, HK_next, qh_next, (float*)nullptr, (int*)nullptr, (int*)nullptr);
    MG_CHECK_LAUNCH("mgnns_label_tail_bf16_fwd");
    return 0;
}
```

mgnns_amd/ops.py:

```python
import os

import torch

from . import _lib
from .derived import derived

ACT_NONE, ACT_RELU, ACT_LRELU2 = 0, 1, 2
BANK_LD = 320


def _stream():
    return torch.cuda.current_stream().cuda_stream


_SCRATCH_EPOCH = 0


def new_scratch_epoch():
    global _SCRATCH_EPOCH
    _SCRATCH_EPOCH += 1
    return _SCRATCH_EPOCH


def set_scratch_epoch(e):
    global _SCRATCH_EPOCH
    prev, _SCRATCH_EPOCH = _SCRATCH_EPOCH, int(e)
    return prev


def _scratch_key():
    return (_SCRATCH_EPOCH, _stream())


_EPOCH_SLOTS = {}


def _scratch_slot_put(slot, key, ws):
    slot[key] = ws
    if key[0]:
        _EPOCH_SLOTS.setdefault(key[0], []).append((slot, key))


def release_scratch_epoch(epoch):
    for slot, key in _EPOCH_SLOTS.pop(int(epoch), []):
        slot.pop(key, None)


_LIVE_CAPTURES = 0
_RETIRED = []


def capture_born():
    global _LIVE_CAPTURES
    _LIVE_CAPTURES += 1


def capture_gone():
    global _LIVE_CAPTURES
    if _LIVE_CAPTURES > 0:
        _LIVE_CAPTURES -= 1
    if _LIVE_CAPTURES == 0:
        _RETIRED.clear()


def retire(obj):
    if obj is not None and _LIVE_CAPTURES > 0:
        _RETIRED.append(obj)


_ZERO_POOL = {}
_ZERO_CHUNK = 64 << 20


def _capturing():
    return torch.cuda.is_current_stream_capturing()


def reserve_zeros(device, nbytes=24 << 20):
    device = torch.device(device)
    pool = _ZERO_POOL.get(device)
    if (pool is None or pool[1] + nbytes > pool[0].numel()) and not _capturing():
        buf = torch.zeros(max(_ZERO_CHUNK, nbytes), dtype=torch.uint8, device=device)
        torch.cuda.current_stream(device).synchronize()
        _ZERO_POOL[device] = [buf, 0]


def zeros_bytes(nbytes, device):
    device = torch.device(device)
    n = (int(nbytes) + 255) // 256 * 256
    pool = _ZERO_POOL.get(device)
    if pool is None or pool[1] + n > pool[0].numel():
        if _capturing():
            return torch.zeros(n, dtype=torch.uint8, device=device)
        reserve_zeros(device, max(n, 24 << 20))
        pool = _ZERO_POOL[device]
    t = pool[0][pool[1]:pool[1] + n]
    pool[1] += n
    return t


def zeros_i32(n, device):
    return zeros_bytes(4 * n, device).view(torch.int32)[:n]


def _scratch_slot(packed, name, fits, make):
    slot = packed.setdefault(name, {})
    key = _scratch_key()
    ws = slot.get(key)
    if ws is None or not fits(ws):
        if ws is not None:
            packed.setdefault("_retired", []).append(ws)
        ws = make()
        _scratch_slot_put(slot, key, ws)
    return key, ws


def _cluster_scratch(packed, name, device, tiles, floats):
    return _scratch_slot(packed, name, lambda ws: ws[0] >= tiles and ws[1].device == device,
                         lambda: (tiles, torch.empty(floats(tiles), device=device, dtype=torch.float32),
                                  zeros_i32(2 * tiles, device)))[1]


class KernelTimer:

    def __init__(self, names=None):
        self.names = None if names is None else set(names)
        self.events = {}

    def wants(self, name):
        return self.names is None or name in self.names

    def durations_ms(self):
        return {k: [a.elapsed_time(b) for a, b in v] for k, v in self.events.items()}


_TIMER = None


def set_timer(timer):
    global _TIMER
    _TIMER = timer


def _launch(name, key, fn, *args):
    t = _TIMER
    if t is not None and t.wants(name):
        a = torch.cuda.Event(enable_timing=True)
        b = torch.cuda.Event(enable_timing=True)
        a.record()
        rc = fn(*args)
        b.record()
        t.events.setdefault(key, []).append((a, b))
    else:
        rc = fn(*args)
    _lib.check(rc, name)


def _chk(t, name, dtype=torch.float32, ndim=None):
    if not torch.is_tensor(t):
        raise TypeError("%s must be a torch tensor" % name)
    if not t.is_cuda:
        raise RuntimeError("%s is on %s: mgnns_amd operators run on the GPU only (no CPU path)" % (name, t.device))
    if t.dtype != dtype:
        raise TypeError("%s must be %s, got %s" % (name, dtype, t.dtype))
    if ndim is not None and t.dim() != ndim:
        raise ValueError("%s must be %d-d, got shape %s" % (name, ndim, tuple(t.shape)))
    if not t.is_contiguous():
        raise ValueError("%s must be contiguous" % name)
    return t


def _p(t):
    return None if t is None else t.data_ptr()


_gemm_ws = {}


def _gemm_workspace(device):
    key = (str(device), torch.cuda.current_stream().cuda_stream)
    buf = _gemm_ws.get(key)
    if buf is None:
        buf = torch.empty(_lib.lib().mgnns_gemm_workspace_bytes(), dtype=torch.uint8, device=device)
        _gemm_ws[key] = buf
    return buf


def linear(x, weight, bias=None, act=ACT_NONE, residual=None):
    K = x.shape[-1]
    x2 = _chk(x.reshape(-1, K), "x")
    _chk(weight, "weight", ndim=2)
    if weight.shape[1] != K:
        raise ValueError("weight %s does not match x[..., %d]" % (tuple(weight.shape), K))
    N = weight.shape[0]
    if bias is not None:
        _chk(bias, "bias", ndim=1)
    y = torch.empty(x2.shape[0], N, device=x.device, dtype=torch.float32)
    if residual is not None:
        residual = _chk(residual.reshape(-1, N), "residual")
        if residual.shape[0] != x2.shape[0]:
            raise ValueError("residual rows mismatch")
    L = _lib.lib()
    ws = _gemm_workspace(x.device)
    _lib.check(L.mgnns_linear_fwd(_p(x2), x2.shape[0], K, _p(weight), _p(bias), N, _p(residual), _p(y), act,
                                  _p(ws), ws.numel(), _stream()), "mgnns_linear_fwd")
    return y.view(*x.shape[:-1], N)


def classifier_head(feats, weight, bias):
    if len(feats) != 4:
        raise ValueError("classifier_head takes the four fusion features")
    B, D = feats[0].shape
    for i, f in enumerate(feats):
        _chk(f, "feature %d" % i, ndim=2)
        if tuple(f.shape) != (B, D):
            raise ValueError("feature %d shape %s, expected %s" % (i, tuple(f.shape), (B, D)))
    _chk(weight, "weight", ndim=2)
    _chk(bias, "bias", ndim=1)
    NL = weight.shape[0]
    if weight.shape[1] != 4 * D or bias.shape[0] != NL:
        raise ValueError("weight %s / bias %s do not match four [B,%d] features" % (tuple(weight.shape), tuple(bias.shape), D))
    out = torch.empty(B, NL, device=weight.device, dtype=torch.float32)
    L = _lib.lib()
    _lib.check(L.mgnns_classifier_head_fwd(_p(feats[0]), _p(feats[1]), _p(feats[2]), _p(feats[3]), B, D, _p(weight), _p(bias), NL,
                                           _p(out), _stream()), "mgnns_classifier_head_fwd")
    return out


def classifier_head_state(B, NL, nparts, device):
    return (torch.empty(nparts, B, NL, device=device, dtype=torch.float32), zeros_i32(1, device),
            torch.empty(B, NL, device=device, dtype=torch.float32))


def classifier_head_part(feat, part, nparts, weight, bias, state):
    _chk(feat, "feature", ndim=2)
    _chk(weight, "weight", ndim=2)
    _chk(bias, "bias", ndim=1)
    B, D = feat.shape
    parts, counter, logits = state
    NL = weight.shape[0]
    if weight.shape[1] != nparts * D or tuple(parts.shape) != (nparts, B, NL) or tuple(logits.shape) != (B, NL):
        raise ValueError("classifier_head_part: weight %s / state do not match %d features [B=%d,%d]" % (tuple(weight.shape), nparts, B, D))
    L = _lib.lib()
    _lib.check(L.mgnns_classifier_part_fwd(_p(feat), int(part), int(nparts), B, D, _p(weight), _p(bias), NL, _p(parts), _p(counter),
                                           _p(logits), _stream()), "mgnns_classifier_part_fwd")
    return logits


def matmul(x, w, act=ACT_NONE):
    _chk(x, "x", ndim=2)
    _chk(w, "w", ndim=2)
    if x.shape[1] != w.shape[0]:
        raise ValueError("matmul shapes %s x %s" % (tuple(x.shape), tuple(w.shape)))
    y = torch.empty(x.shape[0], w.shape[1], device=x.device, dtype=torch.float32)
    L = _lib.lib()
    ws = _gemm_workspace(x.device)
    _lib.check(L.mgnns_matmul_fwd(_p(x), x.shape[0], x.shape[1], _p(w), w.shape[1], _p(y), act, _p(ws), ws.numel(),
                                  _stream()), "mgnns_matmul_fwd")
    return y


def gen_adj(A, want_csr=False):
    _chk(A, "A", ndim=2)
    C = A.shape[0]
    if A.shape[1] != C:
        raise ValueError("A must be square")
    adj = torch.empty_like(A)
    work = torch.empty(C, device=A.device, dtype=torch.float32)
    rp = col = val = None
    if want_csr:
        rp = torch.empty(C + 1, device=A.device, dtype=torch.int32)
        col = torch.empty(C * C, device=A.device, dtype=torch.int32)
        val = torch.empty(C * C, device=A.device, dtype=torch.float32)
    L = _lib.lib()
    _lib.check(L.mgnns_gen_adj(_p(A), C, _p(adj), _p(work), _p(rp), _p(col), _p(val), _stream()), "mgnns_gen_adj")
    return (adj, (rp, col, val)) if want_csr else adj


def label_gcn_pack(w1, w2, split):
    _chk(w1, "gc1.weight", ndim=2)
    _chk(w2, "gc2.weight", ndim=2)
    if w1.shape[1] != w2.shape[0]:
        raise ValueError("gc1.weight %s / gc2.weight %s do not chain" % (tuple(w1.shape), tuple(w2.shape)))
    w1t, w2t = w1.t().contiguous(), w2.t().contiguous()
    if split:
        a, b = pack_weight_bf16_split(w1t), pack_weight_bf16_split(w2t)
        d = {"w1": a, "w2": b}
    else:
        d = {"w1": (pack_weight_f32(w1t), None), "w2": (pack_weight_f32(w2t), None)}
    d.update(split=bool(split), K0=w1.shape[0], N1=w1.shape[1], N2=w2.shape[1])
    return d


LABEL_GCN_GRID = 0


def label_gcn_memo_flag(memo, want_packed_g=False):
    st = memo[_scratch_key() + (bool(want_packed_g),)]
    return int(st["state"][:12].view(torch.int32)[1].item())


def label_gcn(A, inp, packed, want_packed_g=False, query=None, grid=0, memo=None):
    _chk(A, "A", ndim=2)
    _chk(inp, "inp", ndim=2)
    C = A.shape[0]
    if A.shape[1] != C or inp.shape[0] != C or inp.shape[1] != packed["K0"]:
        raise ValueError("A %s / inp %s do not match a [C,C] adjacency and [C,%d] label embeddings" %
                         (tuple(A.shape), tuple(inp.shape), packed["K0"]))
    N1, N2 = packed["N1"], packed["N2"]
    L = _lib.lib()
    need = L.mgnns_label_gcn_scratch_bytes(C, N1, N2)
    key, ws = _scratch_slot(packed, "_scratch", lambda ws: ws.numel() >= need and ws.device == A.device,
                            lambda: zeros_bytes(need, A.device)[:need])
    st = None
    if memo is not None and _TIMER is not None and _TIMER.wants("mgnns_label_gcn_fwd"):
        memo = None
    if memo is not None:
        mkey = key + (bool(want_packed_g),)
        st = memo.get(mkey)
        if st is None:
            mneed = L.mgnns_label_gcn_memo_bytes(C, packed["K0"])
            st = {"state": zeros_bytes(mneed, A.device)[:mneed]}
            _scratch_slot_put(memo, mkey, st)
    if st is not None and "G" in st:
        G, gh, gl = st["G"], st["gh"], st["gl"]
    else:
        G = torch.empty(C, N2, device=A.device, dtype=torch.float32)
        gh = gl = None
        if want_packed_g:
            n = L.mgnns_packed_bf16_weight_bytes(C, N2)
            gh = torch.empty(n, dtype=torch.uint8, device=A.device)
            gl = torch.empty(n, dtype=torch.uint8, device=A.device)
    lq = wq = bq = Q = None
    nlq = hq = 0
    if query is not None:
        lq, wq, bq = query
        _chk(lq, "label_query", ndim=2)
        _chk(wq, "w_q.weight", ndim=2)
        if lq.shape[1] != packed["K0"] or wq.shape[1] != packed["K0"]:
            raise ValueError("label_query %s / w_q.weight %s must be [*, %d]" % (tuple(lq.shape), tuple(wq.shape), packed["K0"]))
        if bq is not None:
            _chk(bq, "w_q.bias", ndim=1)
        nlq, hq = lq.shape[0], wq.shape[0]
        Q = st["Q"] if st is not None and "G" in st else torch.empty(nlq, hq, device=A.device, dtype=torch.float32)
    if st is not None:
        if "G" in st and (Q is None) != (st["Q"] is None):
            raise ValueError("label_gcn: one memo serves one query (present or absent)")
        st.update(G=G, gh=gh, gl=gl, Q=Q)
        mem = st["state"]
        _launch("mgnns_label_gcn_fwd", ("mgnns_label_gcn_fwd", C, packed["split"]), L.mgnns_label_gcn_memo_fwd, _p(A), C, _p(inp),
                packed["K0"], 1 if packed["split"] else 0, _p(packed["w1"][0]), _p(packed["w1"][1]), N1, _p(packed["w2"][0]),
                _p(packed["w2"][1]), N2, _p(G), _p(gh), _p(gl), _p(lq), nlq, _p(wq), _p(bq), hq, _p(Q), _p(ws), ws.numel(), _p(mem),
                mem.numel(), int(grid) or LABEL_GCN_GRID, _stream())
        return G, ((gh, gl) if want_packed_g else None), Q
    _launch("mgnns_label_gcn_fwd", ("mgnns_label_gcn_fwd", C, packed["split"]), L.mgnns_label_gcn_fwd, _p(A), C, _p(inp), packed["K0"],
            1 if packed["split"] else 0, _p(packed["w1"][0]), _p(packed["w1"][1]), N1, _p(packed["w2"][0]), _p(packed["w2"][1]), N2,
            _p(G), _p(gh), _p(gl), _p(lq), nlq, _p(wq), _p(bq), hq, _p(Q), _p(ws), ws.numel(), int(grid) or LABEL_GCN_GRID, _stream())
    return G, ((gh, gl) if want_packed_g else None), Q


def dense_to_csr(m):
    _chk(m, "adj", ndim=2)
    C = m.shape[0]
    if m.shape[1] != C:
        raise ValueError("adj must be square")
    rp = torch.empty(C + 1, device=m.device, dtype=torch.int32)
    col = torch.empty(C * C, device=m.device, dtype=torch.int32)
    val = torch.empty(C * C, device=m.device, dtype=torch.float32)
    L = _lib.lib()
    _lib.check(L.mgnns_dense_to_csr(_p(m), C, _p(rp), _p(col), _p(val), _stream()), "mgnns_dense_to_csr")
    return rp, col, val


def spmm_csr(csr, x, act=ACT_NONE, out=None, bias=None):
    rp, col, val = csr
    _chk(rp, "row_ptr", torch.int32, 1)
    _chk(col, "col", torch.int32, 1)
    _chk(val, "val", torch.float32, 1)
    _chk(x, "x", ndim=2)
    n = rp.shape[0] - 1
    if out is None:
        y = torch.empty(n, x.shape[1], device=x.device, dtype=torch.float32)
    else:
        y = _chk(out, "out", ndim=2)
        if tuple(y.shape) != (n, x.shape[1]) or y.data_ptr() == x.data_ptr():
            raise ValueError("out must be a [%d, %d] tensor distinct from x" % (n, x.shape[1]))
    L = _lib.lib()
    if bias is not None:
        bias = _chk(bias.reshape(-1), "bias", ndim=1)
        if bias.shape[0] != x.shape[1]:
            raise ValueError("bias has %d elements, x has %d features" % (bias.shape[0], x.shape[1]))
        _launch("mgnns_spmm_csr_fwd", ("mgnns_spmm_csr_bias_fwd", n, x.shape[1]), L.mgnns_spmm_csr_bias_fwd, _p(rp), _p(col), _p(val), n,
                _p(x), x.shape[1], _p(bias), _p(y), act, _stream())
        return y
    _launch("mgnns_spmm_csr_fwd", ("mgnns_spmm_csr_fwd", n, x.shape[1]), L.mgnns_spmm_csr_fwd, _p(rp), _p(col), _p(val), n,
            _p(x), x.shape[1], _p(y), act, _stream())
    return y


def cast_bf16(x):
    _chk(x, "x")
    y = torch.empty(x.shape, device=x.device, dtype=torch.bfloat16)
    if x.numel() == 0:
        return y
    _lib.check(_lib.lib().mgnns_cast_bf16(_p(x), x.numel(), _p(y), _stream()), "mgnns_cast_bf16")
    return y


class SparseAdjBf16:

    TILED_MIN_AVG_NNZ = 32.0

    def __init__(self, csr, n_cols=None, sort_rows=True):
        rp, col, val = csr
        _chk(rp, "row_ptr", torch.int32, 1)
        _chk(col, "col", torch.int32, 1)
        if val.dtype == torch.float32:
            val = cast_bf16(_chk(val, "val", torch.float32, 1))
        _chk(val, "val", torch.bfloat16, 1)
        if val.numel() % 2:
            val = torch.cat([val, val.new_zeros(1)])[:-1]
        self.row_ptr, self.col, self.val = rp, col, val
        self.n_rows = rp.shape[0] - 1
# ... 88 lines not shown
    else:
        raise ValueError("path must be None, 'direct' or 'tiled'")
    return y


def embedding(idx, table):
    _chk(idx, "idx", torch.int64)
    _chk(table, "table", ndim=2)
    out = torch.empty(*idx.shape, table.shape[1], device=table.device, dtype=torch.float32)
    L = _lib.lib()
    _lib.check(L.mgnns_embedding_fwd(_p(idx), idx.numel(), _p(table), table.shape[0], table.shape[1], _p(out),
                                     _stream()), "mgnns_embedding_fwd")
    return out


class LstmCache:

    def __init__(self):
        self.cat = None
        self.prepack = None
        self.table = None


def _lstm_derived(cache, slot, sources, build):
    return build() if cache is None else derived(vars(cache), slot, sources, build, park=retire)


def _lstm_cat(weights, num_layers, cache):
    return _lstm_derived(cache, "cat", [t for tup in weights for t in (tup[0], tup[2])], lambda: [
        (torch.cat([weights[2 * l][0], weights[2 * l + 1][0]], 0).contiguous(),
         torch.cat([weights[2 * l][2], weights[2 * l + 1][2]], 0).contiguous()) for l in range(num_layers)])


LSTM_FOLD_EMBEDDING = os.environ.get("MGNNS_LSTM_FOLD", "1") != "0"


def _lstm_table(emb_table, cat0, hidden, cache):
    def build():
        L = _lib.lib()
        V, E = emb_table.shape
        table = torch.empty(V, 8 * hidden, device=emb_table.device, dtype=torch.float32)
        assert table.numel() * 4 == L.mgnns_bilstm_bf16_table_bytes(V, hidden)
        ws = torch.empty(L.mgnns_bilstm_bf16_fold_workspace_bytes(V), dtype=torch.uint8, device=emb_table.device)
        _lib.check(L.mgnns_bilstm_bf16_fold_embedding(_p(emb_table), V, E, hidden, _p(cat0[0]), _p(cat0[1]), _p(ws), ws.numel(),
                                                      _p(table), _stream()), "mgnns_bilstm_bf16_fold_embedding")
        return table
    return _lstm_derived(cache, "table", [emb_table, cat0[0], cat0[1]], build)


def bilstm(tok, lens, emb_table, weights, hidden, num_layers, want_bf16=False, recurrence="f32", cache=None, fold=None):
    import ctypes
    _chk(tok, "text", torch.int64, 2)
    _chk(lens, "text_lens", torch.int64, 1)
    _chk(emb_table, "embedding.weight", ndim=2)
    B, T = tok.shape
    if lens.shape[0] != B:
        raise ValueError("text_lens has %d entries for batch %d" % (lens.shape[0], B))
    if len(weights) != 2 * num_layers:
        raise ValueError("need %d (layer, direction) weight tuples" % (2 * num_layers))
    for li, tup in enumerate(weights):
        in_dim = emb_table.shape[1] if li < 2 else 2 * hidden
        shapes = ((4 * hidden, in_dim), (4 * hidden, hidden), (4 * hidden,), (4 * hidden,))
        for t, shp in zip(tup, shapes):
            _chk(t, "lstm weight")
            if tuple(t.shape) != shp:
                raise ValueError("lstm weight shape %s, expected %s" % (tuple(t.shape), shp))
    cat = _lstm_cat(weights, num_layers, cache)
    arr = lambda ptrs: (ctypes.c_void_p * len(ptrs))(*ptrs)
    c_wih = arr([c[0].data_ptr() for c in cat])
    c_bih = arr([c[1].data_ptr() for c in cat])
    c_whh = arr([w[1].data_ptr() for w in weights])
    c_bhh = arr([w[3].data_ptr() for w in weights])
    L = _lib.lib()
    nbytes = L.mgnns_bilstm_workspace_bytes(B, T, hidden, num_layers)
    ws = torch.empty(max(nbytes, 16), dtype=torch.uint8, device=tok.device)
    out = torch.empty(B, T, 2 * hidden, device=tok.device, dtype=torch.float32)
    out_bf = torch.empty(B, T, BANK_LD, device=tok.device, dtype=torch.bfloat16) if want_bf16 else None
    if recurrence not in ("f32", "bf16"):
        raise ValueError("recurrence must be 'f32' or 'bf16', got %r" % (recurrence,))
    if recurrence == "f32":
        _launch("mgnns_bilstm_fwd", ("mgnns_bilstm_fwd",), L.mgnns_bilstm_fwd, _p(tok), _p(lens), B, T, _p(emb_table),
                emb_table.shape[0], emb_table.shape[1], hidden, num_layers, c_wih, c_bih, c_whh, c_bhh,
                _p(ws), ws.numel(), _p(out), _p(out_bf), BANK_LD, _stream())
    else:
        def prepack():
            pre = torch.empty(L.mgnns_bilstm_bf16_prepack_bytes(hidden, num_layers), dtype=torch.uint8, device=tok.device)
            _lib.check(L.mgnns_bilstm_bf16_prepack(c_wih, c_whh, emb_table.shape[1], hidden, num_layers, _p(pre), _stream()),
                       "mgnns_bilstm_bf16_prepack")
            return pre
        pre = _lstm_derived(cache, "prepack", [t for tup in weights for t in (tup[0], tup[1])], prepack)
        if fold is None:
            fold = LSTM_FOLD_EMBEDDING and cache is not None
        if fold and B <= 1024 and T <= 1024 and emb_table.shape[1] % 4 == 0 and emb_table.shape[1] <= 320:
            table = _lstm_table(emb_table, cat[0], hidden, cache)
            _launch("mgnns_bilstm_bf16_table_fwd", ("mgnns_bilstm_bf16_table_fwd",), L.mgnns_bilstm_bf16_table_fwd, _p(tok), _p(lens), B, T,
                    _p(emb_table), emb_table.shape[0], emb_table.shape[1], hidden, num_layers, c_wih, c_bih, c_whh, c_bhh,
                    _p(ws), ws.numel(), _p(out), _p(out_bf), BANK_LD, _p(pre), _p(table), _stream())
        else:
            _launch("mgnns_bilstm_bf16_fwd", ("mgnns_bilstm_bf16_fwd",), L.mgnns_bilstm_bf16_fwd, _p(tok), _p(lens), B, T, _p(emb_table),
                    emb_table.shape[0], emb_table.shape[1], hidden, num_layers, c_wih, c_bih, c_whh, c_bhh,
                    _p(ws), ws.numel(), _p(out), _p(out_bf), BANK_LD, _p(pre), _stream())
    return (out, out_bf) if want_bf16 else out


def textgcn(tok, node_hidden, edge_w, pmi_dev, ngram, max_length=100):
    _chk(tok, "doc_ids", torch.int64, 2)
    _chk(node_hidden, "node_hidden.weight", ndim=2)
    ew = _chk(edge_w.reshape(-1), "seq_edge_w.weight")
    rp, col, eid = pmi_dev
    _chk(rp, "pmi row_ptr", torch.int32, 1)
    _chk(col, "pmi col", torch.int32, 1)
    if eid is not None:
        _chk(eid, "pmi eid", torch.int32, 1)
        if eid.shape != col.shape:
            raise ValueError("pmi eid and col must have the same length")
    B, T = tok.shape
    V, D = node_hidden.shape
    if rp.shape[0] != V + 1:
        raise ValueError("PMI map has %d rows, vocabulary has %d" % (rp.shape[0] - 1, V))
    out = torch.empty(B, D, device=tok.device, dtype=torch.float32)
    L = _lib.lib()
    _launch("mgnns_textgcn_fwd", ("mgnns_textgcn_fwd",), L.mgnns_textgcn_fwd, _p(tok), B, T, _p(node_hidden), V, D,
            _p(ew), ew.shape[0], _p(rp), _p(col), _p(eid), int(ngram), int(max_length), _p(out), _stream())
    return out


IMGBANK_LDW = 304


def transpose_pad(w, ld):
    _chk(w, "w", ndim=2)
    out = torch.empty(w.shape[1], ld, device=w.device, dtype=torch.float32)
    L = _lib.lib()
    _lib.check(L.mgnns_transpose_pad(_p(w), w.shape[0], w.shape[1], _p(out), ld, _stream()), "mgnns_transpose_pad")
    return out


def imgbank_pool(feat, wt, bias, n_out, want_pool=True):
    _chk(feat, "feature map", ndim=3)
    _chk(wt, "wt", ndim=2)
    B, K, P = feat.shape
    if wt.shape[0] != K:
        raise ValueError("wt rows %d != K %d" % (wt.shape[0], K))
    if bias is not None:
        _chk(bias, "bias", ndim=1)
    bank = torch.empty(B, P, n_out, device=feat.device, dtype=torch.float32)
    pooled = torch.empty(B, K, device=feat.device, dtype=torch.float32) if want_pool else None
    L = _lib.lib()
    _launch("mgnns_imgbank_pool_fwd", ("mgnns_imgbank_pool_fwd",), L.mgnns_imgbank_pool_fwd, _p(feat), B, K, P,
            _p(wt), wt.shape[1], _p(bias), n_out, _p(bank), _p(pooled), _stream())
    return bank, pooled


def pack_imgbank_weights_bf16(w):
    _chk(w, "weight", ndim=2)
    L = _lib.lib()
    buf = torch.empty(L.mgnns_imgbank_packed_weight_bytes(w.shape[1]), dtype=torch.uint8, device=w.device)
    _lib.check(L.mgnns_imgbank_pack_weights_bf16(_p(w), w.shape[0], w.shape[1], _p(buf), _stream()),
               "mgnns_imgbank_pack_weights_bf16")
    return buf


def imgbank_pool_bf16(feat, wp, bias, n_out, combine=True):
    _chk(feat, "feature map", ndim=3)
    _chk(wp, "packed weight", torch.uint8, 1)
    B, K, P = feat.shape
    if bias is not None:
        _chk(bias, "bias", ndim=1)
    bank = torch.empty(B, P, BANK_LD, device=feat.device, dtype=torch.bfloat16)
    pooled = torch.empty(B, K, device=feat.device, dtype=torch.float32)
    work = torch.empty(B, 2, K, device=feat.device, dtype=torch.float32)
    L = _lib.lib()
    _launch("mgnns_imgbank_pool_bf16_fwd", ("mgnns_imgbank_pool_bf16_fwd",), L.mgnns_imgbank_pool_bf16_fwd, _p(feat),
            B, K, P, _p(wp), _p(bias), n_out, _p(bank), BANK_LD, _p(pooled) if combine else None, _p(work), _stream())
    return bank, (pooled if combine else work)


def head_diff(o, n_head):
    _chk(o, "attention output", ndim=2)
    B = o.shape[0]
    if o.shape[1] % n_head:
        raise ValueError("attention output width %d is not a multiple of n_head=%d" % (o.shape[1], n_head))
    out = torch.empty(B, device=o.device, dtype=torch.float32)
    L = _lib.lib()
    _launch("mgnns_head_diff_fwd", ("mgnns_head_diff_fwd",), L.mgnns_head_diff_fwd, _p(o), B, n_head, o.shape[1] // n_head, _p(out),
            _stream())
    return out


def textgcn_set_form(form):
    _lib.check(_lib.lib().mgnns_textgcn_set_form(int(form)), "mgnns_textgcn_set_form")


def imgbank_set_form(form):
    _lib.check(_lib.lib().mgnns_imgbank_set_form(int(form)), "mgnns_imgbank_set_form")


def imgbank_pool_split(feat, w_pair, bias, n_out, want_pool=True, want_f32=True, want_split=False):
    _chk(feat, "feature map", ndim=3)
    B, K, P = feat.shape
    hi, lo = w_pair
    _chk(hi, "packed hi", torch.uint8, 1)
    _chk(lo, "packed lo", torch.uint8, 1)
    if bias is not None:
        _chk(bias, "bias", ndim=1)
    if not (want_f32 or want_split):
        raise ValueError("imgbank_pool_split: nothing to compute (want_f32 or want_split)")
    bank = torch.empty(B, P, n_out, device=feat.device, dtype=torch.float32) if want_f32 else None
    split = torch.empty(2, B, P, BANK_LD, device=feat.device, dtype=torch.bfloat16) if want_split else None
    pooled = torch.empty(B, 2, K, device=feat.device, dtype=torch.float32) if want_pool else None
    L = _lib.lib()
    _launch("mgnns_imgbank_pool_split_fwd", ("mgnns_imgbank_pool_split_fwd", P), L.mgnns_imgbank_pool_split_fwd, _p(feat), B, K, P,
            _p(hi), _p(lo), _p(bias), n_out, _p(bank), _p(pooled), _p(split[0]) if want_split else None,
            _p(split[1]) if want_split else None, _stream())
    return (bank, pooled, split) if want_split else (bank, pooled)


def label_attn_core(Q, K, V, n_heads, mask=None):
    _chk(Q, "Q", ndim=2)
    _chk(K, "K", ndim=2)
    _chk(V, "V", ndim=2)
    NLQ, hid = Q.shape
    B = K.shape[0]
    if K.shape[1] != hid or V.shape != K.shape or hid % n_heads:
        raise ValueError("label attention shapes Q%s K%s V%s" % (tuple(Q.shape), tuple(K.shape), tuple(V.shape)))
    x = torch.empty(B, NLQ, hid, device=K.device, dtype=torch.float32)
    L = _lib.lib()
    if mask is not None:
        if mask.device != K.device:
            raise ValueError("mask is on %s, K on %s" % (mask.device, K.device))
        m8 = torch.broadcast_to(mask != 0, (B, NLQ, n_heads, hid // n_heads)).to(torch.uint8).contiguous()
        _lib.check(L.mgnns_label_attn_core_masked_fwd(_p(Q), _p(K), _p(V), _p(m8), B, NLQ, n_heads, hid // n_heads, _p(x), _stream()),
                   "mgnns_label_attn_core_masked_fwd")
        return x
    _lib.check(L.mgnns_label_attn_core_fwd(_p(Q), _p(K), _p(V), B, NLQ, n_heads, hid // n_heads, _p(x), _stream()),
               "mgnns_label_attn_core_fwd")
    return x


def label_tail(x, Q, n_heads, packed, pooled=None, g_wp=None, next_q=None):
    _chk(Q, "Q", ndim=2)
    NLQ, hid = Q.shape
    if hid % n_heads:
        raise ValueError("hidden width %d is not a multiple of %d heads" % (hid, n_heads))
    if (x is None) == (g_wp is None):
        raise ValueError("pass either x or (pooled, g_wp)")
    parts = kp = 0
    if x is not None:
        _chk(x, "x", ndim=2)
        B, C = x.shape
    else:
        _chk(pooled, "pooled", ndim=3)
        _chk(g_wp, "packed G", ndim=1)
        B, parts, kp = pooled.shape
        C = packed["C"]
    if C != packed["C"]:
        raise ValueError("read-out width %d does not match the packed w_k / w_v (%d)" % (C, packed["C"]))
    for k in ("wk", "wv", "wc", "xl", "bk", "bv", "bc", "bxl"):
        _chk(packed[k], k, ndim=1)
    out = torch.empty(B, packed["n_out"], device=Q.device, dtype=torch.float32)
    wq = bq = qh = None
    hkn = 0
    if next_q is not None:
        wq, bq, hkn = next_q
        qh = torch.empty(B, hkn, device=Q.device, dtype=torch.float32)
    L = _lib.lib()
    _launch("mgnns_label_tail_fwd", ("mgnns_label_tail_fwd", C), L.mgnns_label_tail_fwd, _p(x), B, C, _p(pooled), parts, kp,
            _p(g_wp), _p(Q), NLQ, n_heads, hid // n_heads, _p(packed["wk"]), _p(packed["bk"]), _p(packed["wv"]),
            _p(packed["bv"]), _p(packed["wc"]), _p(packed["bc"]), packed["n5"], _p(packed["xl"]), _p(packed["bxl"]),
            packed["n_out"], _p(out), _p(wq), _p(bq), hkn, _p(qh), _stream())
    return out if next_q is None else (out, qh)


LABEL_TAIL_CLUSTER = True


def label_tail_bf16(pooled, g_pair, Q, n_heads, packed, next_q=None, terms=3, cluster=None):
    import ctypes
    _chk(pooled, "pooled", ndim=3)
    _chk(Q, "Q", ndim=2)
    B, parts, kp = pooled.shape
    NLQ, hid = Q.shape
    if hid % n_heads:
        raise ValueError("hidden width %d is not a multiple of %d heads" % (hid, n_heads))
    pairs = [g_pair, packed["wk"], packed["wv"], packed["wc"], packed["xl"]]
    for k in ("bk", "bv", "bc", "bxl"):
        _chk(packed[k], k, ndim=1)
    out = torch.empty(B, packed["n_out"], device=Q.device, dtype=torch.float32)
    bq = qh = None
    hkn = 0
    if next_q is not None:
        wqp, bq, hkn = next_q
        pairs.append(wqp)
        qh = torch.empty(B, hkn, device=Q.device, dtype=torch.float32)
    ptrs = []
    for h, l in pairs:
        _chk(h, "packed hi", torch.uint8, 1)
        _chk(l, "packed lo", torch.uint8, 1)
        ptrs += [h.data_ptr(), l.data_ptr()]
    ptrs += [None] * (12 - len(ptrs))
    arr = (ctypes.c_void_p * 12)(*ptrs)
    if cluster is None:
        cluster = LABEL_TAIL_CLUSTER
    scratch = counters = None
    if cluster and int(terms) == 3 and B > 0:
        ws = _cluster_scratch(packed, "_cluster_ws", Q.device, (B + 15) // 16, lambda tiles: tiles * 4 * 6144)
        scratch, counters = ws[1], ws[2]
    L = _lib.lib()
    _launch("mgnns_label_tail_bf16_fwd", ("mgnns_label_tail_bf16_fwd", packed["C"]), L.mgnns_label_tail_bf16_fwd, _p(pooled), B,
            parts, kp, packed["C"], int(terms), arr, _p(Q), NLQ, n_heads, hid // n_heads, _p(packed["bk"]), _p(packed["bv"]),
            _p(packed["bc"]), packed["n5"], _p(packed["bxl"]), packed["n_out"], _p(out), _p(bq), hkn, _p(qh), _p(scratch),
            _p(counters), _stream())
    return out if next_q is None else (out, qh)


def sq_mha_core(qh, bank, mask, n_head, d_kv, wk, bk, wv, bv, want_attn=True):
    _chk(qh, "qh", ndim=2)
    _chk(bank, "memory bank", ndim=3)
    B, L_, D = bank.shape
    if qh.shape != (B, n_head * d_kv):
        raise ValueError("qh shape %s, expected %s" % (tuple(qh.shape), (B, n_head * d_kv)))
    if mask is not None:
        _chk(mask, "mask", ndim=2)
        if mask.shape != (B, L_):
            raise ValueError("mask shape %s, expected %s" % (tuple(mask.shape), (B, L_)))
    for n, t in (("w_ks.weight", wk), ("w_vs.weight", wv)):
        _chk(t, n, ndim=2)
        if t.shape != (n_head * d_kv, D):
            raise ValueError("%s shape %s" % (n, tuple(t.shape)))
    o = torch.empty(B, n_head * d_kv, device=bank.device, dtype=torch.float32)
    attn = torch.empty(n_head * B, 1, L_, device=bank.device, dtype=torch.float32) if want_attn else None
    L = _lib.lib()
    _launch("mgnns_sq_mha_core_fwd", ("mgnns_sq_mha_core_fwd", L_, mask is not None), L.mgnns_sq_mha_core_fwd,
            _p(qh), _p(bank), _p(mask), B, L_, D, n_head, d_kv, _p(wk), _p(bk), _p(wv), _p(bv), _p(o), _p(attn),
            _stream())
    return o, attn


MHA_CORE = 32
MHA_CORE_PLAIN = 16
MHA_PACKED = True


def pack_kv_weights_bf16(wk, wv, n_head, d_kv, form=None):
    _chk(wk, "w_ks.weight", ndim=2)
    _chk(wv, "w_vs.weight", ndim=2)
    form = MHA_CORE if form is None else int(form)
    L = _lib.lib()
    if form == 32:
        buf = torch.empty(L.mgnns_sq_mha32_packed_weight_bytes(n_head), dtype=torch.uint8, device=wk.device)
        _lib.check(L.mgnns_sq_mha32_pack_weights_bf16(_p(wk), _p(wv), n_head, d_kv, wk.shape[1], _p(buf), _stream()),
                   "mgnns_sq_mha32_pack_weights_bf16")
    else:
        buf = torch.empty(L.mgnns_sq_mha_packed_weight_bytes(n_head), dtype=torch.uint8, device=wk.device)
        _lib.check(L.mgnns_sq_mha_pack_weights_bf16(_p(wk), _p(wv), n_head, d_kv, wk.shape[1], _p(buf), _stream()),
                   "mgnns_sq_mha_pack_weights_bf16")
    buf._mg_form = form
    return buf


def sq_mha_plan(mask):
    _chk(mask, "mask", ndim=2)
    B, L_ = mask.shape
    if B > PLAN_MAX_B:
        raise ValueError("sq_mha_plan: batch %d beyond the plan kernel's limit %d (fusion.make_mask_plan falls back to the "
                         "one-workgroup-per-sample core)" % (B, PLAN_MAX_B))
    L = _lib.lib()
    plan = torch.empty(L.mgnns_sq_mha32_plan_ints(B), dtype=torch.int32, device=mask.device)
    _lib.check(L.mgnns_sq_mha32_plan(_p(mask), B, L_, _p(plan), _stream()), "mgnns_sq_mha32_plan")
    plan._mg_plan_kind = 'packed'
    return plan


PLAN_MAX_L = 128
PLAN_MAX_B = 4096


def cast_pad_bf16(x, ld=BANK_LD):
    D = x.shape[-1]
    x2 = _chk(x.reshape(-1, D), "x")
    y = torch.empty(x2.shape[0], ld, dtype=torch.bfloat16, device=x.device)
    L = _lib.lib()
    _lib.check(L.mgnns_cast_pad_bf16(_p(x2), x2.shape[0], D, ld, _p(y), _stream()), "mgnns_cast_pad_bf16")
    return y.view(*x.shape[:-1], ld)


def sq_mha_core_bf16(qh, bank_bf16, mask, n_head, d_kv, wp, bk, bv, want_attn=True, plan=None):
    _chk(qh, "qh", ndim=2)
    _chk(bank_bf16, "memory bank (bf16)", torch.bfloat16, 3)
    _chk(wp, "packed K/V weights", torch.uint8, 1)
    B, L_, ld = bank_bf16.shape
    if qh.shape != (B, n_head * d_kv):
        raise ValueError("qh shape %s, expected %s" % (tuple(qh.shape), (B, n_head * d_kv)))
    if mask is not None:
        _chk(mask, "mask", ndim=2)
        if mask.shape != (B, L_):
            raise ValueError("mask shape %s, expected %s" % (tuple(mask.shape), (B, L_)))
    o = torch.empty(B, n_head * d_kv, device=qh.device, dtype=torch.float32)
    attn = torch.empty(n_head * B, 1, L_, device=qh.device, dtype=torch.float32) if want_attn else None
    L = _lib.lib()
    form = getattr(wp, "_mg_form", 16)
    if form == 32:
        if plan is not None:
            _chk(plan, "plan", torch.int32, 1)
            if mask is None or L_ > PLAN_MAX_L or plan.numel() != L.mgnns_sq_mha32_plan_ints(B):
                raise ValueError("a packing plan needs a mask, L <= %d and exactly %d ints (a plan built for this batch size)"
                                 % (PLAN_MAX_L, L.mgnns_sq_mha32_plan_ints(B)))
            if getattr(plan, "_mg_plan_kind", 'packed') != 'packed':
                raise ValueError("sq_mha_core_bf16 takes the plan sq_mha_plan(mask) returned (got kind %r)"
                                 % plan._mg_plan_kind)
        _launch("mgnns_sq_mha_core_bf16_fwd", ("mgnns_sq_mha_core_bf16_fwd", L_, mask is not None),
                L.mgnns_sq_mha32_core_bf16_fwd, _p(qh), _p(bank_bf16), _p(mask), B, L_, ld, n_head, d_kv, _p(wp), _p(bk),
                _p(bv), _p(o), _p(attn), _p(plan), _stream())
        return o, attn
    if plan is not None:
        raise ValueError("a packing plan needs the 32x32x16 form of the packed weights")
    _launch("mgnns_sq_mha_core_bf16_fwd", ("mgnns_sq_mha_core_bf16_fwd", L_, mask is not None),
            L.mgnns_sq_mha_core_bf16_fwd, _p(qh), _p(bank_bf16), _p(mask), B, L_, ld, n_head, d_kv, _p(wp), _p(bk),
            _p(bv), _p(o), _p(attn), _stream())
    return o, attn


def pack_kv_weights_split(wk, wv, n_head, d_kv):
    _chk(wk, "w_ks.weight", ndim=2)
    _chk(wv, "w_vs.weight", ndim=2)
    L = _lib.lib()
    buf = torch.empty(L.mgnns_sq_mha_split_packed_weight_bytes(n_head), dtype=torch.uint8, device=wk.device)
    _lib.check(L.mgnns_sq_mha_pack_weights_split(_p(wk), _p(wv), n_head, d_kv, wk.shape[1], _p(buf), _stream()),
               "mgnns_sq_mha_pack_weights_split")
    buf._mg_form = "split"
    return buf


def split_pad_bf16(x, ld=BANK_LD):
    D = x.shape[-1]
    x2 = _chk(x.reshape(-1, D), "x")
    y = torch.empty(2, x2.shape[0], ld, dtype=torch.bfloat16, device=x.device)
    L = _lib.lib()
    _lib.check(L.mgnns_split_pad_bf16(_p(x2), x2.shape[0], D, ld, _p(y[0]), _p(y[1]), _stream()), "mgnns_split_pad_bf16")
    return y.view(2, *x.shape[:-1], ld)


SPLIT_PLAN_MAX_L = 112


def sq_mha_split_plan(mask):
    _chk(mask, "mask", ndim=2)
    B, L_ = mask.shape
    if B > PLAN_MAX_B or L_ > SPLIT_PLAN_MAX_L:
        raise ValueError("sq_mha_split_plan: B=%d (<= %d), L=%d (<= %d)" % (B, PLAN_MAX_B, L_, SPLIT_PLAN_MAX_L))
    L = _lib.lib()
    plan = torch.empty(L.mgnns_sq_mha32_plan_ints(B), dtype=torch.int32, device=mask.device)
    _lib.check(L.mgnns_sq_mha_split_plan(_p(mask), B, L_, _p(plan), _stream()), "mgnns_sq_mha_split_plan")
    plan._mg_plan_kind = 'grouped'
    return plan


def sq_mha_core_split(qh, bank_split, mask, n_head, d_kv, wp, bk, bv, want_attn=True, plan=None):
    _chk(qh, "qh", ndim=2)
    _chk(bank_split, "memory bank (split bf16)", torch.bfloat16, 4)
    _chk(wp, "packed K/V weights", torch.uint8, 1)
    if getattr(wp, "_mg_form", None) != "split":
        raise ValueError("sq_mha_core_split takes pack_kv_weights_split(...) weights")
    two, B, L_, ld = bank_split.shape
    if two != 2:
        raise ValueError("bank_split must be [2, B, L, %d] (hi, lo)" % BANK_LD)
    if qh.shape != (B, n_head * d_kv):
        raise ValueError("qh shape %s, expected %s" % (tuple(qh.shape), (B, n_head * d_kv)))
    if mask is not None:
        _chk(mask, "mask", ndim=2)
        if mask.shape != (B, L_):
            raise ValueError("mask shape %s, expected %s" % (tuple(mask.shape), (B, L_)))
    o = torch.empty(B, n_head * d_kv, device=qh.device, dtype=torch.float32)
    attn = torch.empty(n_head * B, 1, L_, device=qh.device, dtype=torch.float32) if want_attn else None
    L = _lib.lib()
    if plan is not None:
        _chk(plan, "plan", torch.int32, 1)
        if mask is None or L_ > SPLIT_PLAN_MAX_L or want_attn or plan.numel() != L.mgnns_sq_mha32_plan_ints(B):
            raise ValueError("a group plan needs a mask, L <= %d, want_attn=False and exactly %d ints (a plan built for this batch)"
                             % (SPLIT_PLAN_MAX_L, L.mgnns_sq_mha32_plan_ints(B)))
        if getattr(plan, "_mg_plan_kind", None) != 'grouped':
            raise ValueError("sq_mha_core_split takes the plan sq_mha_split_plan(mask) returned (got kind %r)"
                             % getattr(plan, "_mg_plan_kind", None))
    _launch("mgnns_sq_mha_core_split_fwd", ("mgnns_sq_mha_core_split_fwd", L_, mask is not None), L.mgnns_sq_mha_core_split_fwd,
            _p(qh), _p(bank_split[0]), _p(bank_split[1]), _p(mask), B, L_, ld, n_head, d_kv, _p(wp), _p(bk), _p(bv), _p(o),
            _p(attn), _p(plan), _stream())
    return o, attn


def sq_mha_folded(qh, bank, mask, n_head, d_kv, wk, wv, bv, want_attn=True):
    _chk(qh, "qh", ndim=2)
    is_bf16 = bank.dtype == torch.bfloat16
    _chk(bank, "memory bank", torch.bfloat16 if is_bf16 else torch.float32, 3)
    B, L_, ld = bank.shape
    for n, t in (("w_ks.weight", wk), ("w_vs.weight", wv)):
        _chk(t, n, ndim=2)
    D = wk.shape[1]
    if qh.shape != (B, n_head * d_kv):
        raise ValueError("qh shape %s, expected %s" % (tuple(qh.shape), (B, n_head * d_kv)))
    if wk.shape != (n_head * d_kv, D) or wv.shape != (n_head * d_kv, D):
        raise ValueError("w_ks %s / w_vs %s, expected %s" % (tuple(wk.shape), tuple(wv.shape), (n_head * d_kv, D)))
    if (ld != D) if not is_bf16 else (ld < D):
        raise ValueError("memory bank last dim %d does not match d_model %d" % (ld, D))
    if mask is not None:
        _chk(mask, "mask", ndim=2)
        if mask.shape != (B, L_):
            raise ValueError("mask shape %s, expected %s" % (tuple(mask.shape), (B, L_)))
    o = torch.empty(B, n_head * d_kv, device=qh.device, dtype=torch.float32)
    attn = torch.empty(n_head * B, 1, L_, device=qh.device, dtype=torch.float32) if want_attn else None
    L = _lib.lib()
    nbytes = L.mgnns_sq_mha_folded_workspace_bytes(B, D, n_head)
    ws = torch.empty(max(nbytes, 16), dtype=torch.uint8, device=qh.device)
    _launch("mgnns_sq_mha_folded_fwd", ("mgnns_sq_mha_folded_fwd", L_, is_bf16), L.mgnns_sq_mha_folded_fwd,
            _p(qh), _p(bank), int(is_bf16), ld, _p(mask), B, L_, D, n_head, d_kv, _p(wk), _p(wv), _p(bv), _p(ws), nbytes,
            _p(o), _p(attn), _stream())
    return o, attn


def sq_mha_folded_bf16(u, bank_bf16, mask, n_head, d_kv, want_attn=True):
    _chk(u, "u", ndim=2)
    _chk(bank_bf16, "memory bank", torch.bfloat16, 3)
    B, L_, ld = bank_bf16.shape
    if ld != 320:
        raise ValueError("bf16 memory bank last dim %d, expected 320 (cast_pad_bf16)" % ld)
    if u.shape[0] != B or u.shape[1] % n_head:
        raise ValueError("u shape %s does not match batch %d / %d heads" % (tuple(u.shape), B, n_head))
    D = u.shape[1] // n_head
    if mask is not None:
        _chk(mask, "mask", ndim=2)
        if mask.shape != (B, L_):
            raise ValueError("mask shape %s, expected %s" % (tuple(mask.shape), (B, L_)))
    ldc = (n_head * D + 31) // 32 * 32
    c = torch.empty(B, ldc, device=u.device, dtype=torch.bfloat16)
    attn = torch.empty(n_head * B, 1, L_, device=u.device, dtype=torch.float32) if want_attn else None
    L = _lib.lib()
    _launch("mgnns_sq_mha_folded_bf16_fwd", ("mgnns_sq_mha_folded_bf16_fwd", L_), L.mgnns_sq_mha_folded_bf16_fwd,
            _p(u), _p(bank_bf16), _p(mask), B, L_, D, n_head, float(1.0 / (d_kv ** 0.5)), _p(c), ldc, _p(attn), _stream())
    return c, attn


def pack_weight_f32(w):
    _chk(w, "weight", ndim=2)
    L = _lib.lib()
    buf = torch.empty(L.mgnns_packed_f32_weight_bytes(w.shape[0], w.shape[1]) // 4, dtype=torch.float32, device=w.device)
    _lib.check(L.mgnns_pack_weight_f32(_p(w), w.shape[0], w.shape[1], _p(buf), _stream()), "mgnns_pack_weight_f32")
    return buf


def mha_tail(o, q, packed, eps, next_packed=None):
    _chk(o, "o", ndim=2)
    _chk(q, "q", ndim=2)
    B, HK = o.shape
    if q.shape != (B, 300):
        raise ValueError("q shape %s, expected (%d, 300)" % (tuple(q.shape), B))
    out = torch.empty(B, 300, device=o.device, dtype=torch.float32)
    wq = bq = qh = None
    hkn = 0
    if next_packed is not None:
        wq, bq, hkn = next_packed
        qh = torch.empty(B, hkn, device=o.device, dtype=torch.float32)
    L = _lib.lib()
    _launch("mgnns_mha_tail_fwd", ("mgnns_mha_tail_fwd",), L.mgnns_mha_tail_fwd, _p(o), HK, _p(q), B, 300,
            _p(packed["fc_wp"]), _p(packed["fc_b"]), _p(packed["g1"]), _p(packed["be1"]), _p(packed["w1_wp"]),
            _p(packed["b1"]), _p(packed["w2_wp"]), _p(packed["b2"]), _p(packed["g2"]), _p(packed["be2"]), float(eps),
            _p(out), _p(wq), _p(bq), hkn, _p(qh), _stream())
    return out, qh


def pack_weight_bf16_split(w):
    _chk(w, "weight", ndim=2)
    L = _lib.lib()
    n = L.mgnns_packed_bf16_weight_bytes(w.shape[0], w.shape[1])
    hi = torch.empty(n, dtype=torch.uint8, device=w.device)
    lo = torch.empty(n, dtype=torch.uint8, device=w.device)
    _lib.check(L.mgnns_pack_weight_bf16_split(_p(w), w.shape[0], w.shape[1], _p(hi), _p(lo), _stream()),
               "mgnns_pack_weight_bf16_split")
    return hi, lo


def mha_tail_bf16(o, q, packed, eps, next_packed=None, terms=3, cluster=0, ksplit=True, next_linear=None):
    import ctypes
    _chk(o, "o", ndim=2)
    _chk(q, "q", ndim=2)
    B, HK = o.shape
    if q.shape != (B, 300):
        raise ValueError("q shape %s, expected (%d, 300)" % (tuple(q.shape), B))
    out = torch.empty(B, 300, device=o.device, dtype=torch.float32)
    ptrs = [packed["fc"][0].data_ptr(), packed["fc"][1].data_ptr(), packed["w1"][0].data_ptr(),
            packed["w1"][1].data_ptr(), packed["w2"][0].data_ptr(), packed["w2"][1].data_ptr(), None, None]
    bq = qh = None
    hkn = 0
    use_ks = ksplit and B > 0 and cluster != 1
    if int(terms) == 3 and use_ks and next_packed is not None and next_linear is None:
        use_ks = False
    split_proj = int(terms) == 3 and use_ks and next_linear is not None
    if next_packed is not None and not split_proj:
        (wh, wl), bq, hkn = next_packed
        ptrs[6], ptrs[7] = wh.data_ptr(), wl.data_ptr()
        qh = torch.empty(B, hkn, device=o.device, dtype=torch.float32)
    arr = (ctypes.c_void_p * 8)(*ptrs)
    L = _lib.lib()
    scratch = counters = None
    if use_ks and int(terms) in (1, 3):
        ws = _cluster_scratch(packed, "_cluster_ws_ks", o.device, (B + 15) // 16,
                              lambda tiles: L.mgnns_mha_tail_c16_scratch_floats(16 * tiles, 8))
        scratch, counters = ws[1], ws[2]
    _launch("mgnns_mha_tail_bf16_fwd", ("mgnns_mha_tail_bf16_fwd",), L.mgnns_mha_tail_bf16_fwd, _p(o), HK, _p(q), B, 300,
            int(terms), arr, _p(packed["fc_b"]), _p(packed["g1"]), _p(packed["be1"]), _p(packed["b1"]), _p(packed["b2"]),
            _p(packed["g2"]), _p(packed["be2"]), float(eps), _p(out), _p(bq), hkn, _p(qh), int(cluster), _p(scratch), _p(counters),
            _stream())
    if split_proj:
        qh = linear(out, next_linear[0], next_linear[1])
    return out, qh


# ... 833 lines not shown
```

Measured before the change: 424,300 samples/s.

## Split label-tail middle stages across four cluster ranks with shared scratch exchange

Adds a shared-middle variant of the four-rank label-tail kernel. Each rank now computes only its slice of the K/V projections, the label loop and the output GEMM, and exchanges the partial results through global scratch with extra counter barriers. Before, every rank redundantly computed all of these. The Python wrapper now routes the clustered three-term path to the new entry point. This cuts redundant GEMM work and weight traffic per block, at the cost of more inter-block spin barriers and scratch round trips.

Result: no change. 427,900 samples/s (median of 4 runs) (+0.8%).

```diff
diff --git a/include/mgnns_hip.h b/include/mgnns_hip.h
--- a/include/mgnns_hip.h
+++ b/include/mgnns_hip.h
@@ -127,6 +127,14 @@
                               const float* bv, const float* bc, int N5, const float* bxl, int n_out, float* out,
                               const float* bq_next, int HK_next, float* qh_next, float* cluster_scratch,
                               int* cluster_counters, mgnns_stream_t stream);
+
+size_t mgnns_label_tail_bf16_shared_scratch_bytes(int B);
+size_t mgnns_label_tail_bf16_shared_counters(int B);
+int mgnns_label_tail_bf16_shared_fwd(const float* pooled, int B, int n_parts, int K_pool, int C, const void* const* packed,
+                                     const float* Q, int NLQ, int n_heads, int dh, const float* bk, const float* bv,
+                                     const float* bc, int N5, const float* bxl, int n_out, float* out, const float* bq_next,
+                                     int HK_next, float* qh_next, float* cluster_scratch, size_t scratch_bytes,
+                                     int* cluster_counters, int n_counters, mgnns_stream_t stream);
 
 int mgnns_sq_mha_core_fwd(const float* qh, const float* bank, const float* mask,
                           int B, int L, int D, int H, int dk,
diff --git a/mgnns_amd/_lib.py b/mgnns_amd/_lib.py
--- a/mgnns_amd/_lib.py
+++ b/mgnns_amd/_lib.py
@@ -46,6 +46,8 @@
     "mgnns_label_gcn_memo_fwd": [_P, _I, _P, _I, _I, _P, _P, _I, _P, _P, _I, _P, _P, _P, _P, _I, _P, _P, _I, _P, _P, _SZ, _P, _SZ, _I, _P],
     "mgnns_classifier_head_fwd": [_P, _P, _P, _P, _I, _I, _P, _P, _I, _P, _P],
     "mgnns_label_tail_bf16_fwd": [_P, _I, _I, _I, _I, _I, _PP, _P, _I, _I, _I, _P, _P, _P, _I, _P, _I, _P, _P, _I, _P, _P, _P, _P],
+    "mgnns_label_tail_bf16_shared_fwd": [_P, _I, _I, _I, _I, _PP, _P, _I, _I, _I, _P, _P, _P, _I, _P, _I, _P, _P, _I, _P, _P, _SZ,
+                                         _P, _I, _P],
     "mgnns_label_tail_fwd": [_P, _I, _I, _P, _I, _I, _P, _P, _I, _I, _I, _P, _P, _P, _P, _P, _P, _I, _P, _P, _I, _P, _P, _P,
                              _I, _P, _P],
     "mgnns_sq_mha_core_fwd": [_P, _P, _P, _I, _I, _I, _I, _I, _P, _P, _P, _P, _P, _P, _P],
@@ -144,6 +146,8 @@
     "mgnns_bilstm_bf16_prepack_bytes": [_I, _I],
     "mgnns_bilstm_bf16_table_bytes": [_I, _I],
     "mgnns_bilstm_bf16_fold_workspace_bytes": [_I],
+    "mgnns_label_tail_bf16_shared_scratch_bytes": [_I],
+    "mgnns_label_tail_bf16_shared_counters": [_I],
     "mgnns_label_gcn_scratch_bytes": [_I, _I, _I],
     "mgnns_label_gcn_memo_bytes": [_I, _I],
     "mgnns_mha_tail_c16_scratch_floats": [_I, _I],
diff --git a/mgnns_amd/csrc/label_tail.hip b/mgnns_amd/csrc/label_tail.hip
--- a/mgnns_amd/csrc/label_tail.hip
+++ b/mgnns_amd/csrc/label_tail.hip
@@ -268,7 +268,35 @@
 
 __device__ __forceinline__ unsigned pk2(float a, float b) { return mg_bf16(a) | (unsigned)mg_bf16(b) << 16; }
 
-template <int TERMS, int CL>
+constexpr int LT_XP_BYTES = 8 * 3 * 64 * 16;
+constexpr int LT_KV_TILES = 20;
+constexpr int LT_KV_BYTES = 2 * LT_KV_TILES * 64 * 16;
+constexpr int LT_FL_TILES = 64;
+constexpr int LT_FL_BYTES = LT_FL_TILES * 64 * 16;
+constexpr int LT_OUT_TILES = 24;
+constexpr int LT_OUT_BYTES = LT_OUT_TILES * 64 * 16;
+constexpr int LT_COUNTERS = 2;
+
+__device__ __forceinline__ void lt_arrive_wait(int* ctr, int n, int* status) {
+    __hip_atomic_fetch_add(ctr, 1, __ATOMIC_RELAXED, __HIP_MEMORY_SCOPE_AGENT);
+    int spins = 0;
+    while (__hip_atomic_load(ctr, __ATOMIC_RELAXED, __HIP_MEMORY_SCOPE_AGENT) < n) {
+        if (++spins > (1 << 24)) {
+            if (status) __hip_atomic_store(status, MGNNS_STATUS_CLUSTER_TIMEOUT, __ATOMIC_RELAXED, __HIP_MEMORY_SCOPE_SYSTEM);
+            break;
+        }
+        __builtin_amdgcn_s_sleep(4);
+    }
+}
+
+__device__ __forceinline__ void lt_depart(int* ctr, int ranks) {
+    if (__hip_atomic_fetch_add(&ctr[1], 1, __ATOMIC_RELAXED, __HIP_MEMORY_SCOPE_AGENT) == ranks - 1) {
+        __hip_atomic_store(&ctr[0], 0, __ATOMIC_RELAXED, __HIP_MEMORY_SCOPE_AGENT);
+        __hip_atomic_store(&ctr[1], 0, __ATOMIC_RELAXED, __HIP_MEMORY_SCOPE_AGENT);
+    }
+}
+
+template <int TERMS, int CL, bool SH = false>
 __global__ __launch_bounds__(LT_THR) void label_tail_bf16_kernel(const float* __restrict__ pooled, int B, int n_parts, int KP, int C,
                                                                  const float* __restrict__ Q, int NLQ, int n_heads, int dh,
                                                                  LabelW w, int N5, int NO, float* __restrict__ out, int HKn,
@@ -277,6 +305,7 @@
     extern __shared__ __attribute__((aligned(16))) unsigned char smem_b[];
     constexpr int NH = TERMS == 3 ? 4 : 1;
     constexpr int LO = TERMS == 3 ? 1 : 0;
+    static_assert(!SH || (CL == 4 && TERMS == 3), "the shared middle is a form of the four-rank split-bf16 cluster");
     const int hid = n_heads * dh;
     const int KSp = KP / 32, KSpp = KSp / NH, KSx = (C + 31) / 32, KSh = (hid + 31) / 32, KSf = (NLQ * N5 + 31) / 32;
     const int sp = 4 * KSpp + 2, sxc = 4 * KSx + 2, shc = 4 * KSh + 2, sfc = 4 * KSf + 2;
@@ -317,6 +346,24 @@
 #define MG_LT_PF3 4
 #endif
     WRing<3, TERMS, (TERMS == 3 ? MG_LT_PF3 : 10)> ring;
+    WRing<2, TERMS, 6> ring2;
+    WRing<1, TERMS, 12> ring1;
+    WRing<3, TERMS, (TERMS == 3 ? MG_LT_PF3 : 10)> ringq_;
+    auto& ringq = SH ? ringq_ : ring;
+    f32x4 acc2[2], acc1[1];
+    const int kv_half = (NTh + 1) / 2, kv_sel = crank >> 1;
+    const int kv_lo_ = (crank & 1) * kv_half, kv_n = min(kv_half, NTh - kv_lo_), kv_lo = kv_n > 0 ? kv_lo_ : 0;
+    const int xo_per = (NTo + CL - 1) / CL;
+    const int xo_lo_ = crank * xo_per, xo_n = min(xo_per, NTo - xo_lo_), xo_lo = xo_n > 0 ? xo_lo_ : 0;
+    const unsigned short* kv_h = (kv_sel ? w.wv_h : w.wk_h) + ((size_t)kv_lo * KSx << 9);
+    const unsigned short* kv_l = (kv_sel ? w.wv_l : w.wk_l) + ((size_t)kv_lo * KSx << 9);
+    const unsigned short* xo_h = w.xl_h + ((size_t)xo_lo * KSf << 9);
+    const unsigned short* xo_l = w.xl_l + ((size_t)xo_lo * KSf << 9);
+    const int n_tiles = (int)gridDim.x / CL;
+    unsigned char* kv_scr = reinterpret_cast<unsigned char*>(xpart) + (size_t)n_tiles * CL * LT_XP_BYTES;
+    unsigned char* fl_scr = kv_scr + (size_t)n_tiles * LT_KV_BYTES;
+    unsigned char* out_scr = fl_scr + (size_t)n_tiles * LT_FL_BYTES;
+    const bool lsplit = SH && NLQ * NT5 <= LT_FL_TILES;
     ring_prime(ring, KSpp, w.g_h, w.g_l, NTc, wave, lane, 0, KSp, CL > 1 ? crank * KSpp : 0);
 #if MG_LT_TOUCH
     int touch_sink = 0;
@@ -383,34 +430,28 @@
         __syncthreads();
     }
     LT_STAMP(2);
-    ring_prime(ring, KSx, w.wk_h, w.wk_l, NTh, wave, lane, 0);
+    if constexpr (SH) {
+        if (wave < kv_n) ring_prime(ring2, KSx, kv_h, kv_l, kv_n, wave, lane, 0);
+    } else {
+        ring_prime(ring, KSx, w.wk_h, w.wk_l, NTh, wave, lane, 0);
+    }
     if (CL > 1) {
-        const __amdgpu_buffer_rsrc_t xp = mg_buffer(xpart + (size_t)tile * CL * (8 * 3 * 64 * 4), CL * 8 * 3 * 64 * 16);
+        const __amdgpu_buffer_rsrc_t xp = mg_buffer(xpart + (size_t)tile * CL * (LT_XP_BYTES / 4), CL * LT_XP_BYTES);
         const int slot = (wave * 3 * 64 + lane) * 16;
 #pragma unroll
         for (int t = 0; t < 3; ++t)
             if (wave + 8 * t < NTc)
-                __builtin_amdgcn_raw_buffer_store_b128(__builtin_bit_cast(i32x4, acc[t]), xp, slot + t * 64 * 16, crank * (8 * 3 * 64 * 16), 17);
+                __builtin_amdgcn_raw_buffer_store_b128(__builtin_bit_cast(i32x4, acc[t]), xp, slot + t * 64 * 16, crank * LT_XP_BYTES, 17);
         asm volatile("s_waitcnt vmcnt(0)" ::: "memory");
         __syncthreads();
-        if (tid == 0) {
-            __hip_atomic_fetch_add(&counters[2 * tile], 1, __ATOMIC_RELAXED, __HIP_MEMORY_SCOPE_AGENT);
-            int spins = 0;
-            while (__hip_atomic_load(&counters[2 * tile], __ATOMIC_RELAXED, __HIP_MEMORY_SCOPE_AGENT) < CL) {
-                if (++spins > (1 << 24)) {
-                    if (status) __hip_atomic_store(status, MGNNS_STATUS_CLUSTER_TIMEOUT, __ATOMIC_RELAXED, __HIP_MEMORY_SCOPE_SYSTEM);
-                    break;
-                }
-                __builtin_amdgcn_s_sleep(4);
-            }
-        }
+        if (tid == 0) lt_arrive_wait(&counters[LT_COUNTERS * tile], CL, status);
         __syncthreads();
 #pragma unroll
         for (int t = 0; t < 3; ++t) {
             f32x4 pr[CL];
 #pragma unroll
             for (int rk = 0; rk < CL; ++rk)
-                pr[rk] = wave + 8 * t < NTc ? __builtin_bit_cast(f32x4, __builtin_amdgcn_raw_buffer_load_b128(xp, slot + t * 64 * 16, rk * (8 * 3 * 64 * 16), 17))
+                pr[rk] = wave + 8 * t < NTc ? __builtin_bit_cast(f32x4, __builtin_amdgcn_raw_buffer_load_b128(xp, slot + t * 64 * 16, rk * LT_XP_BYTES, 17))
                                             : f32x4{0.f, 0.f, 0.f, 0.f};
             acc[t] = pr[0];
 #pragma unroll
@@ -427,34 +468,45 @@
     }
     for (int i = tid; i < (1 + LO) * LT_ROWS * spf; i += LT_THR) s_ph[i] = make_uint4(0u, 0u, 0u, 0u);
     __syncthreads();
-    if (CL > 1 && tid == 0) {
-        const int old = __hip_atomic_fetch_add(&counters[2 * tile + 1], 1, __ATOMIC_RELAXED, __HIP_MEMORY_SCOPE_AGENT);
-        if (old == CL - 1) {
-            __hip_atomic_store(&counters[2 * tile], 0, __ATOMIC_RELAXED, __HIP_MEMORY_SCOPE_AGENT);
-            __hip_atomic_store(&counters[2 * tile + 1], 0, __ATOMIC_RELAXED, __HIP_MEMORY_SCOPE_AGENT);
-        }
-    }
+    if (CL > 1 && !SH && tid == 0) lt_depart(&counters[LT_COUNTERS * tile], CL);
     LT_STAMP(3);
-    ring_gemm(acc, ring, s_xh, s_xl, sxc, KSx, w.wk_h, w.wk_l, lane);
-    ring_prime(ring, KSx, w.wv_h, w.wv_l, NTh, wave, lane, 0);
-#pragma unroll
-    for (int t = 0; t < 3; ++t) {
-        const int nt = wave + 8 * t, n = nt * 16 + ccol;
-        if (nt < NTh && n < hid) {
-            const float b0 = w.bk[n];
-#pragma unroll
-            for (int r = 0; r < 4; ++r) s_k[(crow + r) * shf + n] = acc[t][r] + b0;
-        }
-    }
-    ring_gemm(acc, ring, s_xh, s_xl, sxc, KSx, w.wv_h, w.wv_l, lane);
-    ring_prime(ring, KSf, w.xl_h, w.xl_l, NTo, wave, lane, 0);
-#pragma unroll
-    for (int t = 0; t < 3; ++t) {
-        const int nt = wave + 8 * t, n = nt * 16 + ccol;
-        if (nt < NTh && n < hid) {
-            const float b0 = w.bv[n];
-#pragma unroll
-            for (int r = 0; r < 4; ++r) s_v[(crow + r) * shf + n] = acc[t][r] + b0;
+    if constexpr (SH) {
+        const __amdgpu_buffer_rsrc_t kvb = mg_buffer(kv_scr + (size_t)tile * LT_KV_BYTES, LT_KV_BYTES);
+        if (wave < kv_n) ring_gemm(acc2, ring2, s_xh, s_xl, sxc, KSx, kv_h, kv_l, lane);
+        if (wave < xo_n) ring_prime(ring1, KSf, xo_h, xo_l, xo_n, wave, lane, 0);
+        LT_STAMP(8);
+        const float* bkv = kv_sel ? w.bv : w.bk;
+#pragma unroll
+        for (int t = 0; t < 2; ++t) {
+            const int nt = kv_lo + wave + 8 * t, n = nt * 16 + ccol;
+            if (wave + 8 * t < kv_n) {
+                const float b0 = n < hid ? bkv[n] : 0.f;
+                const f32x4 v = {acc2[t][0] + b0, acc2[t][1] + b0, acc2[t][2] + b0, acc2[t][3] + b0};
+                __builtin_amdgcn_raw_buffer_store_b128(__builtin_bit_cast(i32x4, v), kvb, ((kv_sel * LT_KV_TILES + nt) * 64 + lane) * 16, 0, 17);
+            }
+        }
+    } else {
+        ring_gemm(acc, ring, s_xh, s_xl, sxc, KSx, w.wk_h, w.wk_l, lane);
+        ring_prime(ring, KSx, w.wv_h, w.wv_l, NTh, wave, lane, 0);
+#pragma unroll
+        for (int t = 0; t < 3; ++t) {
+            const int nt = wave + 8 * t, n = nt * 16 + ccol;
+            if (nt < NTh && n < hid) {
+                const float b0 = w.bk[n];
+#pragma unroll
+                for (int r = 0; r < 4; ++r) s_k[(crow + r) * shf + n] = acc[t][r] + b0;
+            }
+        }
+        ring_gemm(acc, ring, s_xh, s_xl, sxc, KSx, w.wv_h, w.wv_l, lane);
+        ring_prime(ring, KSf, w.xl_h, w.xl_l, NTo, wave, lane, 0);
+#pragma unroll
+        for (int t = 0; t < 3; ++t) {
+            const int nt = wave + 8 * t, n = nt * 16 + ccol;
+            if (nt < NTh && n < hid) {
+                const float b0 = w.bv[n];
+#pragma unroll
+                for (int r = 0; r < 4; ++r) s_v[(crow + r) * shf + n] = acc[t][r] + b0;
+            }
         }
     }
     uint4 wch[LB_MAXKS], wcl[LO ? LB_MAXKS : 1];
@@ -466,11 +518,41 @@
             if (LO) wcl[ks] = reinterpret_cast<const uint4*>(w.wc_l)[off];
         }
     }
+    if constexpr (SH) {
+        const __amdgpu_buffer_rsrc_t kvb = mg_buffer(kv_scr + (size_t)tile * LT_KV_BYTES, LT_KV_BYTES);
+        asm volatile("s_waitcnt vmcnt(0)" ::: "memory");
+        __syncthreads();
+        if (tid == 0) {
+            lt_arrive_wait(&counters[LT_COUNTERS * tile], 2 * CL, status);
+            if (!w.wq_h && !lsplit) lt_depart(&counters[LT_COUNTERS * tile], CL);
+        }
+        __syncthreads();
+        constexpr int NJ = 2 * LT_KV_TILES * 64 / LT_THR;
+        f32x4 kvv[NJ];
+#pragma unroll
+        for (int j = 0; j < NJ; ++j) {
+            const int sl = tid + LT_THR * j, kv = sl >= NTh * 64, rem = sl - kv * NTh * 64;
+            kvv[j] = sl < 2 * NTh * 64 ? __builtin_bit_cast(f32x4, __builtin_amdgcn_raw_buffer_load_b128(kvb, ((kv * LT_KV_TILES) * 64 + rem) * 16, 0, 17))
+                                       : f32x4{0.f, 0.f, 0.f, 0.f};
+        }
+#pragma unroll
+        for (int j = 0; j < NJ; ++j) {
+            const int sl = tid + LT_THR * j, kv = sl >= NTh * 64, rem = sl - kv * NTh * 64;
+            const int n = (rem >> 6) * 16 + (rem & 15), row = ((rem & 63) >> 4) * 4;
+            if (sl < 2 * NTh * 64 && n < hid) {
+                float* dst = (kv ? s_v : s_k) + row * shf + n;
+#pragma unroll
+                for (int r = 0; r < 4; ++r) dst[r * shf] = kvv[j][r];
+            }
+        }
+    }
     __syncthreads();
 
     const float inv_scale = 1.0f / sqrtf((float)dh);
     LT_STAMP(4);
-    for (int l = 0; l < NLQ; ++l) {
+    const int l_per = (NLQ + CL - 1) / CL;
+    const int l_lo = lsplit ? min(NLQ, crank * l_per) : 0, l_hi = lsplit ? min(NLQ, l_lo + l_per) : NLQ;
+    for (int l = l_lo; l < l_hi; ++l) {
 #pragma unroll 1
         for (int rr = 0; rr < 2; ++rr) {
             const int r = 2 * wave + rr;
@@ -508,7 +590,15 @@
                     }
                 }
             const int n = wave * 16 + ccol;
-            if (n < N5) {
+            if constexpr (SH) {
+                if (lsplit) {
+                    const float b0 = n < N5 ? w.bc[n] : 0.f;
+                    const f32x4 v = {a[0] + b0, a[1] + b0, a[2] + b0, a[3] + b0};
+                    __builtin_amdgcn_raw_buffer_store_b128(__builtin_bit_cast(i32x4, v), mg_buffer(fl_scr + (size_t)tile * LT_FL_BYTES, LT_FL_BYTES),
+                                                           ((l * NT5 + wave) * 64 + lane) * 16, 0, 17);
+                }
+            }
+            if (!lsplit && n < N5) {
                 const float b0 = w.bc[n];
 #pragma unroll
                 for (int r = 0; r < 4; ++r) put(fh16, fl16, (crow + r) * sfc * 8 + l * N5 + n, a[r] + b0);
@@ -517,23 +607,98 @@
         __syncthreads();
     }
 
+    if constexpr (SH) {
+        if (lsplit) {
+            const __amdgpu_buffer_rsrc_t fb = mg_buffer(fl_scr + (size_t)tile * LT_FL_BYTES, LT_FL_BYTES);
+            LT_STAMP(10);
+            asm volatile("s_waitcnt vmcnt(0)" ::: "memory");
+            __syncthreads();
+            if (tid == 0) {
+                lt_arrive_wait(&counters[LT_COUNTERS * tile], 3 * CL, status);
+                if (!w.wq_h) lt_depart(&counters[LT_COUNTERS * tile], CL);
+            }
+            __syncthreads();
+            const int nsl = NLQ * NT5 * 64;
+            for (int s0 = 0; s0 < nsl; s0 += 4 * LT_THR) {
+                f32x4 fv[4];
+#pragma unroll
+                for (int j = 0; j < 4; ++j) {
+                    const int sl = s0 + tid + LT_THR * j;
+                    fv[j] = sl < nsl ? __builtin_bit_cast(f32x4, __builtin_amdgcn_raw_buffer_load_b128(fb, sl * 16, 0, 17)) : f32x4{0.f, 0.f, 0.f, 0.f};
+                }
+#pragma unroll
+                for (int j = 0; j < 4; ++j) {
+                    const int sl = s0 + tid + LT_THR * j, lt = sl >> 6, l = lt / NT5, n = (lt - l * NT5) * 16 + (sl & 15), row = ((sl & 63) >> 4) * 4;
+                    if (sl < nsl && n < N5) {
+#pragma unroll
+                        for (int r = 0; r < 4; ++r) put(fh16, fl16, (row + r) * sfc * 8 + l * N5 + n, fv[j][r]);
+                    }
+                }
+            }
+            __syncthreads();
+        }
+    }
     LT_STAMP(5);
-    ring_gemm(acc, ring, s_fh, s_fl, sfc, KSf, w.xl_h, w.xl_l, lane);
+    if constexpr (SH) {
+        if (wave < xo_n) ring_gemm(acc1, ring1, s_fh, s_fl, sfc, KSf, xo_h, xo_l, lane);
+    } else {
+        ring_gemm(acc, ring, s_fh, s_fl, sfc, KSf, w.xl_h, w.xl_l, lane);
+    }
     LT_STAMP(6);
     const int q_slots = ((HKn + 15) / 16 + 7) / 8, q_per = (q_slots + CL - 1) / CL;
     const int q_lo = crank * q_per, q_hi = q_lo + q_per < q_slots ? q_lo + q_per : q_slots;
-    if (w.wq_h) ring_prime(ring, KSh, w.wq_h, w.wq_l, (HKn + 15) / 16, wave, lane, q_lo);
-#pragma unroll
-    for (int t = 0; t < 3; ++t) {
-        const int nt = wave + 8 * t, n = nt * 16 + ccol;
-        if (nt < NTo && n < NO) {
-            const float b0 = w.bxl[n];
+    if (w.wq_h) ring_prime(ringq, KSh, w.wq_h, w.wq_l, (HKn + 15) / 16, wave, lane, q_lo);
+    if constexpr (SH) {
+        const __amdgpu_buffer_rsrc_t ob = mg_buffer(out_scr + (size_t)tile * LT_OUT_BYTES, LT_OUT_BYTES);
+        if (wave < xo_n) {
+            const int nt = xo_lo + wave, n = nt * 16 + ccol;
+            const float b0 = n < NO ? w.bxl[n] : 0.f;
+            const f32x4 v = {acc1[0][0] + b0, acc1[0][1] + b0, acc1[0][2] + b0, acc1[0][3] + b0};
 #pragma unroll
             for (int r = 0; r < 4; ++r) {
                 const int gr = r0 + crow + r;
-                const float v = acc[t][r] + b0;
-                if (gr < B && crank == 0) out[(size_t)gr * NO + n] = v;
-                if (w.wq_h) put(oh16, ol16, (crow + r) * shc * 8 + n, v);
+                if (gr < B && n < NO) out[(size_t)gr * NO + n] = v[r];
+            }
+            if (w.wq_h) __builtin_amdgcn_raw_buffer_store_b128(__builtin_bit_cast(i32x4, v), ob, (nt * 64 + lane) * 16, 0, 17);
+        }
+        if (w.wq_h) {
+            asm volatile("s_waitcnt vmcnt(0)" ::: "memory");
+            __syncthreads();
+            if (tid == 0) {
+                lt_arrive_wait(&counters[LT_COUNTERS * tile], (lsplit ? 4 : 3) * CL, status);
+                lt_depart(&counters[LT_COUNTERS * tile], CL);
+            }
+            __syncthreads();
+            constexpr int NJ = LT_OUT_TILES * 64 / LT_THR;
+            f32x4 ov[NJ];
+#pragma unroll
+            for (int j = 0; j < NJ; ++j) {
+                const int sl = tid + LT_THR * j;
+                ov[j] = sl < NTo * 64 ? __builtin_bit_cast(f32x4, __builtin_amdgcn_raw_buffer_load_b128(ob, sl * 16, 0, 17)) : f32x4{0.f, 0.f, 0.f, 0.f};
+            }
+#pragma unroll
+            for (int j = 0; j < NJ; ++j) {
+                const int sl = tid + LT_THR * j, n = (sl >> 6) * 16 + (sl & 15), row = ((sl & 63) >> 4) * 4;
+                if (sl < NTo * 64 && n < NO) {
+#pragma unroll
+                    for (int r = 0; r < 4; ++r) put(oh16, ol16, (row + r) * shc * 8 + n, ov[j][r]);
+                }
+            }
+        }
+        LT_STAMP(9);
+    } else {
+#pragma unroll
+        for (int t = 0; t < 3; ++t) {
+            const int nt = wave + 8 * t, n = nt * 16 + ccol;
+            if (nt < NTo && n < NO) {
+                const float b0 = w.bxl[n];
+#pragma unroll
+                for (int r = 0; r < 4; ++r) {
+                    const int gr = r0 + crow + r;
+                    const float v = acc[t][r] + b0;
+                    if (gr < B && crank == 0) out[(size_t)gr * NO + n] = v;
+                    if (w.wq_h) put(oh16, ol16, (crow + r) * shc * 8 + n, v);
+                }
             }
         }
     }
@@ -541,8 +706,8 @@
         __syncthreads();
         const int NTq = (HKn + 15) / 16;
         for (int t0 = q_lo; t0 < q_hi; t0 += 3) {
-            if (t0 != q_lo) ring_prime(ring, KSh, w.wq_h, w.wq_l, NTq, wave, lane, t0);
-            ring_gemm(acc, ring, s_oh, s_ol, shc, KSh, w.wq_h, w.wq_l, lane);
+            if (t0 != q_lo) ring_prime(ringq, KSh, w.wq_h, w.wq_l, NTq, wave, lane, t0);
+            ring_gemm(acc, ringq, s_oh, s_ol, shc, KSh, w.wq_h, w.wq_l, lane);
 #pragma unroll
             for (int t = 0; t < 3; ++t) {
                 const int nt = wave + 8 * (t0 + t), n = nt * 16 + ccol;
@@ -580,25 +745,25 @@
     return lds <= 160 * 1024 ? 1 : 0;
 }
 
-extern "C" int mgnns_label_tail_bf16_fwd(const float* pooled, int B, int n_parts, int K_pool, int C, int terms,
-                                         const void* const* packed ,
-                                         const float* Q, int NLQ, int n_heads, int dh, const float* bk, const float* bv,
-                                         const float* bc, int N5, const float* bxl, int n_out, float* out,
-                                         const float* bq_next, int HK_next, float* qh_next, float* cluster_scratch,
-                                         int* cluster_counters, mgnns_stream_t stream) {
+static int lt_bf16_launch(const char* who, bool shared, const float* pooled, int B, int n_parts, int K_pool, int C, int terms,
+                          const void* const* packed ,
+                          const float* Q, int NLQ, int n_heads, int dh, const float* bk, const float* bv,
+                          const float* bc, int N5, const float* bxl, int n_out, float* out,
+                          const float* bq_next, int HK_next, float* qh_next, float* cluster_scratch,
+                          int* cluster_counters, mgnns_stream_t stream) {
     MG_REQUIRE(B >= 0 && C > 0 && C <= 384 && NLQ > 0 && n_heads > 0 && dh > 0 && dh <= 64 && N5 > 0 && N5 <= 128 && n_out > 0,
-               "mgnns_label_tail_bf16_fwd: bad dims B=%d C=%d (<= 384) NLQ=%d heads=%d dh=%d N5=%d out=%d", B, C, NLQ, n_heads, dh, N5, n_out);
-    MG_REQUIRE(terms == 1 || terms == 3, "mgnns_label_tail_bf16_fwd: terms must be 1 (bf16) or 3 (split-bf16)");
+               "%s: bad dims B=%d C=%d (<= 384) NLQ=%d heads=%d dh=%d N5=%d out=%d", who, B, C, NLQ, n_heads, dh, N5, n_out);
+    MG_REQUIRE(terms == 1 || terms == 3, "%s: terms must be 1 (bf16) or 3 (split-bf16)", who);
     if (B == 0) return 0;
-    MG_REQUIRE(pooled && packed && Q && bk && bv && bc && bxl && out, "mgnns_label_tail_bf16_fwd: null pointer");
-    for (int i = 0; i < 10; ++i) MG_REQUIRE(packed[i], "mgnns_label_tail_bf16_fwd: packed weight %d missing", i);
+    MG_REQUIRE(pooled && packed && Q && bk && bv && bc && bxl && out, "%s: null pointer", who);
+    for (int i = 0; i < 10; ++i) MG_REQUIRE(packed[i], "%s: packed weight %d missing", who, i);
     MG_REQUIRE(n_parts >= 1 && K_pool > 0 && K_pool % 128 == 0 && mg_aligned16(pooled),
-               "mgnns_label_tail_bf16_fwd: pooled [B,%d,%d] must be 16-byte aligned with K %% 128 == 0", n_parts, K_pool);
+               "%s: pooled [B,%d,%d] must be 16-byte aligned with K %% 128 == 0", who, n_parts, K_pool);
     const int hid = n_heads * dh;
     MG_REQUIRE(hid <= 32 * LB_MAXKS && n_out <= 384 && n_heads <= LT_MAXH,
-               "mgnns_label_tail_bf16_fwd: hidden width %d / output width %d / %d heads unsupported", hid, n_out, n_heads);
+               "%s: hidden width %d / output width %d / %d heads unsupported", who, hid, n_out, n_heads);
     MG_REQUIRE(!packed[10] || (packed[11] && qh_next && HK_next > 0 && n_out == hid),
-               "mgnns_label_tail_bf16_fwd: the query projection needs both packed buffers, qh_next, HK_next and n_out == hidden width");
+               "%s: the query projection needs both packed buffers, qh_next, HK_next and n_out == hidden width", who);
     LabelW w;
     const unsigned short* const* pk = reinterpret_cast<const unsigned short* const*>(packed);
     w.g_h = pk[0]; w.g_l = pk[1]; w.wk_h = pk[2]; w.wk_l = pk[3]; w.wv_h = pk[4]; w.wv_l = pk[5]; w.wc_h = pk[6]; w.wc_l = pk[7];
@@ -608,17 +773,21 @@
     const int sp = 4 * (K_pool / 32 / nh) + 2, sxc = 4 * ((C + 31) / 32) + 2, shc = 4 * ((hid + 31) / 32) + 2, sfc = 4 * ((NLQ * N5 + 31) / 32) + 2;
     const size_t lds = (size_t)(1 + lo) * LT_ROWS * ((sp > sfc ? sp : sfc) + sxc + shc) * 16 +
                        ((size_t)2 * LT_ROWS * lt_stride(hid) + (size_t)NLQ * hid) * sizeof(float);
-    MG_REQUIRE(lds <= 160 * 1024, "mgnns_label_tail_bf16_fwd: K_pool=%d, C=%d need %zu B of LDS (> 160 KiB)", K_pool, C, lds);
-    MG_REQUIRE((cluster_scratch != nullptr) == (cluster_counters != nullptr), "mgnns_label_tail_bf16_fwd: cluster scratch and counters go together");
-    MG_REQUIRE(!cluster_scratch || mg_aligned16(cluster_scratch), "mgnns_label_tail_bf16_fwd: cluster scratch must be 16-byte aligned");
+    MG_REQUIRE(lds <= 160 * 1024, "%s: K_pool=%d, C=%d need %zu B of LDS (> 160 KiB)", who, K_pool, C, lds);
+    MG_REQUIRE((cluster_scratch != nullptr) == (cluster_counters != nullptr), "%s: cluster scratch and counters go together", who);
+    MG_REQUIRE(!cluster_scratch || mg_aligned16(cluster_scratch), "%s: cluster scratch must be 16-byte aligned", who);
     if (cluster_scratch)
-        if (int rc = mg_check_status("mgnns_label_tail_bf16_fwd")) return rc;
+        if (int rc = mg_check_status(who)) return rc;
     MG_DYN_LDS((label_tail_bf16_kernel<1, 1>), 160 * 1024);
     MG_DYN_LDS((label_tail_bf16_kernel<3, 1>), 160 * 1024);
     MG_DYN_LDS((label_tail_bf16_kernel<3, 4>), 160 * 1024);
+    MG_DYN_LDS((label_tail_bf16_kernel<3, 4, true>), 160 * 1024);
     const int tiles = (B + LT_ROWS - 1) / LT_ROWS;
     const dim3 blk(LT_THR);
-    if (terms == 3 && cluster_scratch)
+    if (terms == 3 && cluster_scratch && shared)
+        hipLaunchKernelGGL((label_tail_bf16_kernel<3, 4, true>), dim3(tiles * 4), blk, lds, (hipStream_t)stream, pooled, B, n_parts, K_pool, C, Q, NLQ,
+                           n_heads, dh, w, N5, n_out, out, HK_next, qh_next, cluster_scratch, cluster_counters, mg_status_word());
+    else if (terms == 3 && cluster_scratch)
         hipLaunchKernelGGL((label_tail_bf16_kernel<3, 4>), dim3(tiles * 4), blk, lds, (hipStream_t)stream, pooled, B, n_parts, K_pool, C, Q, NLQ,
                            n_heads, dh, w, N5, n_out, out, HK_next, qh_next, cluster_scratch, cluster_counters, mg_status_word());
     else if (terms == 3)
@@ -627,6 +796,42 @@
     else
         hipLaunchKernelGGL((label_tail_bf16_kernel<1, 1>), dim3(tiles), blk, lds, (hipStream_t)stream, pooled, B, n_parts, K_pool, C, Q, NLQ, n_heads, dh,
                            w, N5, n_out, out, HK_next, qh_next, (float*)nullptr, (int*)nullptr, (int*)nullptr);
-    MG_CHECK_LAUNCH("mgnns_label_tail_bf16_fwd");
+    MG_CHECK_LAUNCH(who);
     return 0;
 }
+
+extern "C" int mgnns_label_tail_bf16_fwd(const float* pooled, int B, int n_parts, int K_pool, int C, int terms,
+                                         const void* const* packed, const float* Q, int NLQ, int n_heads, int dh, const float* bk,
+                                         const float* bv, const float* bc, int N5, const float* bxl, int n_out, float* out,
+                                         const float* bq_next, int HK_next, float* qh_next, float* cluster_scratch,
+                                         int* cluster_counters, mgnns_stream_t stream) {
+    return lt_bf16_launch("mgnns_label_tail_bf16_fwd", false, pooled, B, n_parts, K_pool, C, terms, packed, Q, NLQ, n_heads, dh, bk, bv, bc, N5,
+                          bxl, n_out, out, bq_next, HK_next, qh_next, cluster_scratch, cluster_counters, stream);
+}
+
+extern "C" size_t mgnns_label_tail_bf16_shared_scratch_bytes(int B) {
+    const size_t tiles = B > 0 ? ((size_t)B + LT_ROWS - 1) / LT_ROWS : 0;
+    return tiles * (4 * LT_XP_BYTES + LT_KV_BYTES + LT_FL_BYTES + LT_OUT_BYTES);
+}
+
+extern "C" size_t mgnns_label_tail_bf16_shared_counters(int B) {
+    const size_t tiles = B > 0 ? ((size_t)B + LT_ROWS - 1) / LT_ROWS : 0;
+    return tiles * LT_COUNTERS;
+}
+
+extern "C" int mgnns_label_tail_bf16_shared_fwd(const float* pooled, int B, int n_parts, int K_pool, int C, const void* const* packed,
+                                                const float* Q, int NLQ, int n_heads, int dh, const float* bk, const float* bv,
+                                                const float* bc, int N5, const float* bxl, int n_out, float* out, const float* bq_next,
+                                                int HK_next, float* qh_next, float* cluster_scratch, size_t scratch_bytes,
+                                                int* cluster_counters, int n_counters, mgnns_stream_t stream) {
+    const char* who = "mgnns_label_tail_bf16_shared_fwd";
+    MG_REQUIRE(B >= 0, "%s: bad batch size %d", who, B);
+    MG_REQUIRE(cluster_scratch && cluster_counters, "%s: the cluster scratch and counters are mandatory", who);
+    MG_REQUIRE(mg_aligned16(cluster_scratch), "%s: cluster scratch must be 16-byte aligned", who);
+    MG_REQUIRE(scratch_bytes >= mgnns_label_tail_bf16_shared_scratch_bytes(B), "%s: scratch of %zu B is too small for B=%d (%zu B)", who,
+               scratch_bytes, B, mgnns_label_tail_bf16_shared_scratch_bytes(B));
+    MG_REQUIRE(n_counters >= 0 && (size_t)n_counters >= mgnns_label_tail_bf16_shared_counters(B), "%s: %d counters are too few for B=%d (%zu)",
+               who, n_counters, B, mgnns_label_tail_bf16_shared_counters(B));
+    return lt_bf16_launch(who, true, pooled, B, n_parts, K_pool, C, 3, packed, Q, NLQ, n_heads, dh, bk, bv, bc, N5, bxl, n_out, out, bq_next,
+                          HK_next, qh_next, cluster_scratch, cluster_counters, stream);
+}
diff --git a/mgnns_amd/ops.py b/mgnns_amd/ops.py
--- a/mgnns_amd/ops.py
+++ b/mgnns_amd/ops.py
@@ -115,10 +115,10 @@
     return key, ws
 
 
-def _cluster_scratch(packed, name, device, tiles, floats):
+def _cluster_scratch(packed, name, device, tiles, floats, counters=None):
     return _scratch_slot(packed, name, lambda ws: ws[0] >= tiles and ws[1].device == device,
                          lambda: (tiles, torch.empty(floats(tiles), device=device, dtype=torch.float32),
-                                  zeros_i32(2 * tiles, device)))[1]
+                                  zeros_i32(counters(tiles) if counters else 2 * tiles, device)))[1]
 
 
 class KernelTimer:
@@ -813,15 +813,20 @@
     arr = (ctypes.c_void_p * 12)(*ptrs)
     if cluster is None:
         cluster = LABEL_TAIL_CLUSTER
-    scratch = counters = None
+    L = _lib.lib()
+    key = ("mgnns_label_tail_bf16_fwd", packed["C"])
     if cluster and int(terms) == 3 and B > 0:
-        ws = _cluster_scratch(packed, "_cluster_ws", Q.device, (B + 15) // 16, lambda tiles: tiles * 4 * 6144)
-        scratch, counters = ws[1], ws[2]
-    L = _lib.lib()
-    _launch("mgnns_label_tail_bf16_fwd", ("mgnns_label_tail_bf16_fwd", packed["C"]), L.mgnns_label_tail_bf16_fwd, _p(pooled), B,
-            parts, kp, packed["C"], int(terms), arr, _p(Q), NLQ, n_heads, hid // n_heads, _p(packed["bk"]), _p(packed["bv"]),
-            _p(packed["bc"]), packed["n5"], _p(packed["bxl"]), packed["n_out"], _p(out), _p(bq), hkn, _p(qh), _p(scratch),
-            _p(counters), _stream())
+        ws = _cluster_scratch(packed, "_cluster_ws", Q.device, (B + 15) // 16,
+                              lambda tiles: L.mgnns_label_tail_bf16_shared_scratch_bytes(16 * tiles) // 4,
+                              lambda tiles: L.mgnns_label_tail_bf16_shared_counters(16 * tiles))
+        _launch("mgnns_label_tail_bf16_fwd", key, L.mgnns_label_tail_bf16_shared_fwd, _p(pooled), B, parts, kp, packed["C"], arr,
+                _p(Q), NLQ, n_heads, hid // n_heads, _p(packed["bk"]), _p(packed["bv"]), _p(packed["bc"]), packed["n5"],
+                _p(packed["bxl"]), packed["n_out"], _p(out), _p(bq), hkn, _p(qh), _p(ws[1]), 4 * ws[1].numel(), _p(ws[2]),
+                ws[2].numel(), _stream())
+    else:
+        _launch("mgnns_label_tail_bf16_fwd", key, L.mgnns_label_tail_bf16_fwd, _p(pooled), B, parts, kp, packed["C"], int(terms),
+                arr, _p(Q), NLQ, n_heads, hid // n_heads, _p(packed["bk"]), _p(packed["bv"]), _p(packed["bc"]), packed["n5"],
+                _p(packed["bxl"]), packed["n_out"], _p(out), _p(bq), hkn, _p(qh), None, None, _stream())
     return out if next_q is None else (out, qh)
 
 
```
